# ekimb/mapquik

Hardware: AMD Instinct MI355X
Metric: Gbases/s mapped (sim CHM13v2-like HiFi, k=5 l=31 d=0.01) (higher is better)
Workload: dtype u64

## Files before the change

include/mapquik_hip_diag.h:

```cpp
#ifndef MAPQUIK_HIP_DIAG_H
#define MAPQUIK_HIP_DIAG_H

#include "mapquik_hip.h"

#ifdef __cplusplus
extern "C" {
#endif

int mq_last_map_path_counts(mq_index *idx, uint32_t *n_fast, uint32_t *n_general);

int mqdiag_last_map_spec(mq_index *idx, uint32_t *spec_id);
int mqdiag_ctx_last_map_spec(mq_ctx *ctx, uint32_t *spec_id);

int mq_last_map_order(mq_index *idx, uint32_t *n_flagged, uint32_t *n_first);

int mq_index_table_alloc_ms(mq_index *idx, float *ms);

int mq_map_launch_waves(mq_index *idx, uint32_t n_reads, uint32_t *n_waves);

int mq_map_probe_stats(mq_index *idx, const uint8_t *d_bases, const uint64_t *d_offsets, uint32_t n, uint64_t total_bases, mq_hit *d_out,
                       uint64_t *lookups, uint64_t *extra_steps);

int mq_last_read_cycles(mq_index *idx, uint32_t n, uint32_t *cycles, uint64_t *start_ticks);

int mq_probe_rate(mq_index *idx, uint32_t blocks, uint32_t per_thread, uint32_t bitmap_log2, uint32_t table_too, float *ms,
                  uint64_t *lookups, uint64_t *extra_steps);

int mq_last_stage_clocks(mq_index *idx, uint64_t *out16);

int mq_last_map_ms(mq_index *idx, float *ms);
int mq_ctx_last_map_ms(mq_ctx *ctx, float *ms);

uint64_t mqdiag_coverage_tile_bits(void);
uint64_t mqdiag_coverage_held(const mq_index *idx);
int mqdiag_coverage_ms(float *out6);

#ifdef __cplusplus
}
#endif

#endif
```

mapquik_amd/api.py:

```python
import ctypes as C
import os

import numpy as np

from . import build as _build

MQ_HIT_UNMAPPED, MQ_HIT_MAPPED, MQ_HIT_OVERFLOW = 0, 1, 2
MQ_FLAG_FOLD_CASE = 1
MQ_FLAG_FAST_KH = 2
MQ_FLAG_SEED_VARIANT_SHIFT = 8
MQ_ABI_VERSION = 4

hit_dtype = np.dtype([("status", "<u4"), ("ref_id", "<u4"), ("rc", "<u4"), ("mapq", "<u4"), ("q_start", "<u4"), ("q_end", "<u4"),
                      ("r_start", "<u4"), ("r_end", "<u4"), ("score", "<u4"), ("n_kminmers", "<u4"), ("q_start_hi", "<u4"), ("q_end_hi", "<u4")])
kminmer_dtype = np.dtype([("hash", "<u8"), ("start", "<u4"), ("end", "<u4"), ("offset", "<u4"), ("rev", "<u4")])
assert hit_dtype.itemsize == 48 and kminmer_dtype.itemsize == 24
anchor_dtype = np.dtype([("q_start", "<u4"), ("q_end", "<u4"), ("r_start", "<u4"), ("r_end", "<u4"), ("count", "<u4")])
anchor_span_dtype = np.dtype([("first", "<u4"), ("count", "<u4")])
MQ_ANCHORS_DROPPED = 0xFFFFFFFF
assert anchor_dtype.itemsize == 20 and anchor_span_dtype.itemsize == 8
chain_dtype = np.dtype([("flags", "<u4"), ("ref_id", "<u4"), ("rc", "<u4"), ("mapq", "<u4"), ("q_start", "<u4"), ("q_end", "<u4"),
                        ("r_start", "<u4"), ("r_end", "<u4"), ("score", "<u4"), ("n_runs", "<u4"), ("q_start_hi", "<u4"), ("q_end_hi", "<u4")])
chain_span_dtype = np.dtype([("first", "<u4"), ("count", "<u4")])
MQ_CHAIN_TOP = 1
# ... 104 lines not shown
    if hasattr(L, "mq_ctx_submit_fasta"):
        L.mq_host_register.argtypes = [vp, C.c_size_t]
        L.mq_host_unregister.argtypes = [vp]
        L.mq_ctx_submit_fasta.argtypes = [vp, vp, u64, u64]
        L.mq_ctx_wait_fasta.argtypes = [vp, C.POINTER(u32), C.POINTER(vp), C.POINTER(u32), C.POINTER(vp), C.POINTER(u32)]
    if hasattr(L, "mq_ctx_submit_fastx"):
        L.mq_ctx_submit_fastx.argtypes = [vp, vp, u64, u64, u32]
    if hasattr(L, "mq_ctx_wait_fasta_lines"):
        L.mq_ctx_wait_fasta_lines.argtypes = [vp, C.POINTER(u32), C.POINTER(vp), C.POINTER(vp), C.POINTER(vp), C.POINTER(vp), C.POINTER(u32)]
    if hasattr(L, "mq_index_stage_begin"):
        L.mq_index_set_table_factor.argtypes = [vp, u32]
        L.mq_index_get_params.argtypes = [vp, C.POINTER(Params)]
        L.mq_index_set_map_params.argtypes = [vp, u32, u32, u32, C.c_int]
        L.mq_index_stage_begin.argtypes = [vp, u64]
        L.mq_index_stage_piece.argtypes = [vp, u64, vp, u64, C.POINTER(u64)]
        L.mq_index_stage_done.argtypes = [vp, u64, C.c_int]
        L.mq_index_add_ref_staged.restype = C.c_int64
        L.mq_index_add_ref_staged.argtypes = [vp, u32, C.c_char_p, u64, u64, u64]
    if hasattr(L, "mq_index_add_ref_staged_lines"):
        L.mq_index_add_ref_staged_lines.restype = C.c_int64
        L.mq_index_add_ref_staged_lines.argtypes = [vp, u32, C.c_char_p, u64, u64, u64, C.POINTER(u64)]
        L.mq_index_staged_sequence.restype = C.c_int64
        L.mq_index_staged_sequence.argtypes = [vp, u64, u64, u64, vp, u64]
    L.mq_ctx_reserve.argtypes = [vp, u32, u64]
    L.mq_ctx_map_batch_device.argtypes = [vp, vp, vp, u32, u64, vp, vp]
    L.mq_ctx_last_map_ms.argtypes = [vp, C.POINTER(C.c_float)]
    L.mq_probe_rate.argtypes = [vp, u32, u32, u32, u32, C.POINTER(C.c_float), C.POINTER(u64), C.POINTER(u64)]
    L.mq_kminmers_batch.argtypes = [vp, vp, vp, u32, vp, vp, vp]
    L.mq_index_lookup.argtypes = [vp, vp, u32, vp, vp, vp]
    L.mq_format_paf.argtypes = [vp, C.c_char_p, u64, vp, C.c_char_p, C.c_size_t]
    L.mq_last_map_ms.argtypes = [vp, C.POINTER(C.c_float)]
    L.mq_last_stage_clocks.argtypes = [vp, vp]
    if hasattr(L, "mq_last_read_cycles"):
        L.mq_last_read_cycles.argtypes = [vp, u32, vp, vp]
    L.mq_map_probe_stats.argtypes = [vp, vp, vp, u32, u64, vp, C.POINTER(u64), C.POINTER(u64)]
    if hasattr(L, "mq_map_launch_waves"):
        L.mq_map_launch_waves.argtypes = [vp, u32, C.POINTER(u32)]
        L.mq_index_table_alloc_ms.argtypes = [vp, C.POINTER(C.c_float)]
    L.mq_index_save.argtypes = [vp, C.c_char_p]
    L.mq_index_clone.restype = vp
    L.mq_index_clone.argtypes = [vp, C.c_int]
    L.mq_index_load.restype = vp
    L.mq_index_load.argtypes = [C.c_char_p, C.c_int]
    L.mq_host_alloc.restype = vp
    L.mq_host_alloc.argtypes = [C.c_size_t]
    L.mq_host_free.argtypes = [vp]
    L.mq_last_map_path_counts.argtypes = [vp, C.POINTER(C.c_uint32), C.POINTER(C.c_uint32)]
    L.mq_last_map_order.argtypes = [vp, C.POINTER(C.c_uint32), C.POINTER(C.c_uint32)]
    if hasattr(L, "mq_ctx_reserve_redo"):
        L.mq_ctx_reserve_redo.argtypes = [vp, u32, u32]
        L.mq_map_reserve_redo.argtypes = [vp, u32, u32]
        L.mq_ctx_redo_counts.argtypes = [vp, C.POINTER(u32), C.POINTER(u32)]
        L.mq_map_redo_counts.argtypes = [vp, C.POINTER(u32), C.POINTER(u32)]
    pp = C.POINTER(vp)
    for kind in ("anchors", "chains"):
        if hasattr(L, "mq_ctx_reserve_" + kind):
            for scope in ("ctx", "map"):
                getattr(L, "mq_%s_reserve_%s" % (scope, kind)).argtypes = [vp, u32, u64]
                getattr(L, "mq_%s_%s" % (scope, kind)).argtypes = [vp, pp, pp, C.POINTER(u32), C.POINTER(u64), C.POINTER(u64), C.POINTER(u32)]
            getattr(L, "mq_ctx_%s_device" % kind).argtypes = [vp, pp, pp]
    if hasattr(L, "mq_format_paf_chain"):
        L.mq_format_paf_chain.argtypes = [vp, C.c_char_p, u64, vp, C.c_char_p, C.c_size_t]
    if hasattr(L, "mq_index_reopen"):
        L.mq_index_reopen.argtypes = [vp]
        L.mq_index_resize.argtypes = [vp, u64, u32]
        L.mq_index_load_sized.restype = vp
        L.mq_index_load_sized.argtypes = [C.c_char_p, C.c_int, u64, u32]
        L.mq_index_clone_sized.restype = vp
        L.mq_index_clone_sized.argtypes = [vp, C.c_int, u64, u32]
    if hasattr(L, "mq_index_merge"):
        L.mq_index_merge.argtypes = [vp, vp, u32]
        L.mq_index_merge_file.argtypes = [vp, C.c_char_p, u32]
    if hasattr(L, "mq_index_coverage"):
        L.mq_index_coverage.argtypes = [vp, C.POINTER(vp), C.POINTER(u64), C.POINTER(vp), C.POINTER(u64), C.POINTER(u64)]
        L.mq_index_coverage_release.argtypes = [vp]
        L.mqdiag_coverage_tile_bits.restype = u64
        L.mqdiag_coverage_tile_bits.argtypes = []
        L.mqdiag_coverage_held.restype = u64
        L.mqdiag_coverage_held.argtypes = [vp]
        L.mqdiag_coverage_ms.argtypes = [C.POINTER(C.c_float)]
    if hasattr(L, "mqdiag_last_map_spec"):
        L.mqdiag_last_map_spec.argtypes = [vp, C.POINTER(C.c_uint32)]
        L.mqdiag_ctx_last_map_spec.argtypes = [vp, C.POINTER(C.c_uint32)]
    if path is None:
        _lib = L
    return L


def _err(L, what):
    return MapquikError("%s: %s" % (what, (L.mq_last_error() or b"").decode(errors="replace")))


def _pooled(L, what, handle, span_dtype, item_dtype):
    sp, it = C.c_void_p(), C.c_void_p()
    n, dropped = C.c_uint32(), C.c_uint32()
    stored, needed = C.c_uint64(), C.c_uint64()
    if getattr(L, what)(handle, C.byref(sp), C.byref(it), C.byref(n), C.byref(stored), C.byref(needed), C.byref(dropped)) != 0:
        raise _err(L, what)
    spans = np.frombuffer(C.string_at(sp.value, n.value * span_dtype.itemsize), dtype=span_dtype).copy() if n.value else np.zeros(0, dtype=span_dtype)
    items = np.frombuffer(C.string_at(it.value, stored.value * item_dtype.itemsize), dtype=item_dtype).copy() if stored.value else np.zeros(0, dtype=item_dtype)
    return spans, items, dict(stored=stored.value, needed=needed.value, dropped_reads=dropped.value)


def _reserve_pooled(L, what, handle, max_reads, max_entries):
    if getattr(L, what)(handle, int(max_reads), int(max_entries)) != 0:
        raise _err(L, what)


def _pooled_device(L, what, handle):
    sp, it = C.c_void_p(), C.c_void_p()
    if getattr(L, what)(handle, C.byref(sp), C.byref(it)) != 0:
        raise _err(L, what)
    return sp.value, it.value


class PinnedBuffer:

    def __init__(self, nbytes):
        self._L = load_library()
        self._p = self._L.mq_host_alloc(nbytes)
        if not self._p:
            raise _err(self._L, "mq_host_alloc")
        self.array = np.ctypeslib.as_array((C.c_uint8 * nbytes).from_address(self._p))

    def close(self):
        if getattr(self, "_p", None):
            self.array = None
            self._L.mq_host_free(self._p)
            self._p = None

    __del__ = close


def device_count():
    return load_library().mq_device_count()


def _seq(seq):
    if isinstance(seq, (bytes, bytearray, memoryview)):
        return np.frombuffer(bytes(seq), dtype=np.uint8)
    return np.ascontiguousarray(seq, dtype=np.uint8)


def _p(a):
    return a.ctypes.data_as(C.c_void_p)


class Index:

    def __init__(self, params=None, device=0, _handle=None):
        self._L = load_library()
        self.params = params or Params()
        self._h = _handle if _handle is not None else self._L.mq_index_new(C.byref(self.params), device)
        if not self._h:
            raise _err(self._L, "mq_index_new")
        self.device = device

    def save(self, path):
        if self._L.mq_index_save(self._h, os.fsencode(path)) != 0:
            raise _err(self._L, "mq_index_save")

    @classmethod
    def load(cls, path, device=0, table_slots=0, factor=0):
        L = load_library()
        if table_slots or factor:
            h, what = L.mq_index_load_sized(os.fsencode(path), device, int(table_slots), int(factor)), "mq_index_load_sized"
# ... 183 lines not shown
        rc = self._L.mq_map_batch_device(self._h, C.c_void_p(d_bases), C.c_void_p(d_offsets), n, int(total_bases), C.c_void_p(d_out),
                                         C.c_void_p(stream))
        if rc != 0:
            raise _err(self._L, "mq_map_batch_device")

    def reserve(self, n_reads, total_bases):
        if self._L.mq_map_reserve(self._h, n_reads, int(total_bases)) != 0:
            raise _err(self._L, "mq_map_reserve")

    def reserve_redo(self, max_reads, max_read_len):
        if self._L.mq_map_reserve_redo(self._h, int(max_reads), int(max_read_len)) != 0:
            raise _err(self._L, "mq_map_reserve_redo")

    def redo_counts(self):
        a, b = C.c_uint32(), C.c_uint32()
        if self._L.mq_map_redo_counts(self._h, C.byref(a), C.byref(b)) != 0:
            raise _err(self._L, "mq_map_redo_counts")
        return a.value, b.value

    def reserve_anchors(self, max_reads, max_anchors):
        _reserve_pooled(self._L, "mq_map_reserve_anchors", self._h, max_reads, max_anchors)

    def anchors(self):
        return _pooled(self._L, "mq_map_anchors", self._h, anchor_span_dtype, anchor_dtype)

    def reserve_chains(self, max_reads, max_chains):
        _reserve_pooled(self._L, "mq_map_reserve_chains", self._h, max_reads, max_chains)

    def chains(self):
        return _pooled(self._L, "mq_map_chains", self._h, chain_span_dtype, chain_dtype)

    def format_paf_chain(self, q_id, q_len, chain):
        rec = np.zeros(1, dtype=chain_dtype)
        rec[0] = chain
        cap = 4096
        while True:
            buf = C.create_string_buffer(cap)
            w = self._L.mq_format_paf_chain(self._h, q_id.encode(), int(q_len), _p(rec), buf, cap)
            if w < 0:
                raise _err(self._L, "mq_format_paf_chain")
            if w < cap:
                return buf.value.decode()
            cap = w + 1

    def context(self):
        return Context(self)

    def last_map_ms(self):
        ms = C.c_float()
        if self._L.mq_last_map_ms(self._h, C.byref(ms)) != 0:
            raise _err(self._L, "mq_last_map_ms")
        return ms.value

    def last_stage_clocks(self):
        out = (C.c_uint64 * 16)()
        if self._L.mq_last_stage_clocks(self._h, out) != 0:
            raise _err(self._L, "mq_last_stage_clocks")
        return [int(x) for x in out]

    def probe_stats(self, d_bases, d_offsets, n, total_bases, d_out):
        a, b = C.c_uint64(), C.c_uint64()
        if self._L.mq_map_probe_stats(self._h, C.c_void_p(d_bases), C.c_void_p(d_offsets), n, int(total_bases), C.c_void_p(d_out),
                                      C.byref(a), C.byref(b)) != 0:
            raise _err(self._L, "mq_map_probe_stats")
        return a.value, b.value

    def probe_rate(self, blocks, per_thread, bitmap_log2=0, table_too=1):
        ms, a, b = C.c_float(), C.c_uint64(), C.c_uint64()
        if self._L.mq_probe_rate(self._h, blocks, per_thread, bitmap_log2, table_too, C.byref(ms), C.byref(a), C.byref(b)) != 0:
            raise _err(self._L, "mq_probe_rate")
        return ms.value, a.value, b.value

    def last_map_path_counts(self):
        a, b = C.c_uint32(), C.c_uint32()
        if self._L.mq_last_map_path_counts(self._h, C.byref(a), C.byref(b)) != 0:
            raise _err(self._L, "mq_last_map_path_counts")
        return a.value, b.value

    def last_map_spec(self):
        a = C.c_uint32()
        if self._L.mqdiag_last_map_spec(self._h, C.byref(a)) != 0:
            raise _err(self._L, "mqdiag_last_map_spec")
        return a.value

    def table_alloc_ms(self):
        ms = C.c_float()
        if self._L.mq_index_table_alloc_ms(self._h, C.byref(ms)) != 0:
            raise _err(self._L, "mq_index_table_alloc_ms")
        return ms.value

    def launch_waves(self, n_reads):
        a = C.c_uint32()
        if self._L.mq_map_launch_waves(self._h, int(n_reads), C.byref(a)) != 0:
            raise _err(self._L, "mq_map_launch_waves")
        return a.value

    def last_map_order(self):
        a, b = C.c_uint32(), C.c_uint32()
        if self._L.mq_last_map_order(self._h, C.byref(a), C.byref(b)) != 0:
            raise _err(self._L, "mq_last_map_order")
        return a.value, b.value

    def kminmers_batch(self, bases, offsets, caps=None):
        bases = _seq(bases)
        offsets = np.ascontiguousarray(offsets, dtype=np.uint64)
        n = offsets.size - 1
        if caps is None:
            caps = (offsets[1:] - offsets[:-1]).astype(np.uint64)
        koff = np.zeros(n + 1, dtype=np.uint64)
        koff[1:] = np.cumsum(np.asarray(caps, dtype=np.uint64))
        out = np.zeros(int(koff[-1]), dtype=kminmer_dtype)
        counts = np.zeros(n, dtype=np.uint32)
        if n > 0 and self._L.mq_kminmers_batch(self._h, _p(bases), _p(offsets), n, _p(koff), _p(out), _p(counts)) != 0:
            raise _err(self._L, "mq_kminmers_batch")
        res = []
        for i in range(n):
            c = int(counts[i])
            if c > int(koff[i + 1] - koff[i]):
                raise MapquikError("k-min-mer window too small for sequence %d: %d > %d" % (i, c, int(koff[i + 1] - koff[i])))
            res.append(out[int(koff[i]):int(koff[i]) + c].copy())
        return res

    def lookup(self, hashes):
        h = np.ascontiguousarray(hashes, dtype=np.uint64)
        n = h.size
        found = np.zeros(n, dtype=np.uint8)
        ent = np.zeros(n, dtype=kminmer_dtype)
        ids = np.zeros(n, dtype=np.uint32)
        if n > 0 and self._L.mq_index_lookup(self._h, _p(h), n, _p(found), _p(ent), _p(ids)) != 0:
            raise _err(self._L, "mq_index_lookup")
        return found, ent, ids

    def format_paf(self, q_id, q_len, hit):
        rec = np.zeros(1, dtype=hit_dtype)
        rec[0] = hit
        cap = 4096
        while True:
            buf = C.create_string_buffer(cap)
            w = self._L.mq_format_paf(self._h, q_id.encode(), int(q_len), _p(rec), buf, cap)
            if w < 0:
                raise _err(self._L, "mq_format_paf")
            if w < cap:
                return buf.value.decode()
            cap = w + 1

    def paf_lines(self, names, offsets, hits):
        out = []
        for i, name in enumerate(names):
            st = int(hits[i]["status"])
            if st == MQ_HIT_OVERFLOW:
                raise MapquikError("read %s: Match-run scratch overflow (raise MQ_MATCH_CAP)" % name)
            if st == MQ_HIT_MAPPED:
                out.append(self.format_paf(name, int(offsets[i + 1] - offsets[i]), hits[i]))
        return out


class Context:

    def __init__(self, index):
        self._L = index._L
        self._index = index
        self._h = self._L.mq_ctx_new(index.handle)
        if not self._h:
            raise _err(self._L, "mq_ctx_new")
        self._keep = None

# ... 40 lines not shown
            if self._L.mq_ctx_submit_fastx(self._h, _p(buf), int(begin), buf.size, 1 if fastq else 2) != 0:
                raise _err(self._L, "mq_ctx_submit_fastx")
        elif self._L.mq_ctx_submit_fasta(self._h, _p(buf), int(begin), buf.size) != 0:
            raise _err(self._L, "mq_ctx_submit_fasta")
        self._keep = (buf,)

    def wait_fasta(self):
        n, nl, fl = C.c_uint32(), C.c_uint32(), C.c_uint32()
        le, hp = C.c_void_p(), C.c_void_p()
        if self._L.mq_ctx_wait_fasta(self._h, C.byref(n), C.byref(le), C.byref(nl), C.byref(hp), C.byref(fl)) != 0:
            raise _err(self._L, "mq_ctx_wait_fasta")
        self._keep = None
        if fl.value & 1 or n.value == 0:
            return np.zeros(0, dtype=hit_dtype), np.zeros(0, dtype=np.uint32), fl.value
        hits = np.frombuffer(C.string_at(hp.value, n.value * hit_dtype.itemsize), dtype=hit_dtype).copy()
        lines = np.frombuffer(C.string_at(le.value, nl.value * 4), dtype=np.uint32).copy()
        return hits, lines, fl.value

    def wait_fasta_lines(self):
        n, fl = C.c_uint32(), C.c_uint32()
        hb, he, sl, hp = C.c_void_p(), C.c_void_p(), C.c_void_p(), C.c_void_p()
        if self._L.mq_ctx_wait_fasta_lines(self._h, C.byref(n), C.byref(hb), C.byref(he), C.byref(sl), C.byref(hp), C.byref(fl)) != 0:
            raise _err(self._L, "mq_ctx_wait_fasta_lines")
        self._keep = None
        if fl.value & 1 or n.value == 0:
            e = np.zeros(0, dtype=np.uint32)
            return np.zeros(0, dtype=hit_dtype), e, e.copy(), e.copy(), fl.value
        hits = np.frombuffer(C.string_at(hp.value, n.value * hit_dtype.itemsize), dtype=hit_dtype).copy()
        u = [np.frombuffer(C.string_at(q.value, n.value * 4), dtype=np.uint32).copy() for q in (hb, he, sl)]
        return hits, u[0], u[1], u[2], fl.value

    def wait(self):
        if self._L.mq_ctx_wait(self._h) != 0:
            raise _err(self._L, "mq_ctx_wait")
        out = self._keep[2] if self._keep else np.zeros(0, dtype=hit_dtype)
        self._keep = None
        return out

    def map_batch_device(self, d_bases, d_offsets, n, total_bases, d_out, stream=0):
        if self._L.mq_ctx_map_batch_device(self._h, C.c_void_p(d_bases), C.c_void_p(d_offsets), n, int(total_bases), C.c_void_p(d_out),
                                           C.c_void_p(stream)) != 0:
            raise _err(self._L, "mq_ctx_map_batch_device")

    def reserve_redo(self, max_reads, max_read_len):
        if self._L.mq_ctx_reserve_redo(self._h, int(max_reads), int(max_read_len)) != 0:
            raise _err(self._L, "mq_ctx_reserve_redo")

    def redo_counts(self):
        a, b = C.c_uint32(), C.c_uint32()
        if self._L.mq_ctx_redo_counts(self._h, C.byref(a), C.byref(b)) != 0:
            raise _err(self._L, "mq_ctx_redo_counts")
        return a.value, b.value

    def reserve_anchors(self, max_reads, max_anchors):
        _reserve_pooled(self._L, "mq_ctx_reserve_anchors", self._h, max_reads, max_anchors)

    def anchors(self):
        return _pooled(self._L, "mq_ctx_anchors", self._h, anchor_span_dtype, anchor_dtype)

    def reserve_chains(self, max_reads, max_chains):
        _reserve_pooled(self._L, "mq_ctx_reserve_chains", self._h, max_reads, max_chains)

    def chains(self):
        return _pooled(self._L, "mq_ctx_chains", self._h, chain_span_dtype, chain_dtype)

    def chains_device(self):
        return _pooled_device(self._L, "mq_ctx_chains_device", self._h)

    def anchors_device(self):
        return _pooled_device(self._L, "mq_ctx_anchors_device", self._h)

    def last_map_ms(self):
        ms = C.c_float()
        if self._L.mq_ctx_last_map_ms(self._h, C.byref(ms)) != 0:
            raise _err(self._L, "mq_ctx_last_map_ms")
        return ms.value

    def last_map_spec(self):
        a = C.c_uint32()
        if self._L.mqdiag_ctx_last_map_spec(self._h, C.byref(a)) != 0:
            raise _err(self._L, "mqdiag_ctx_last_map_spec")
        return a.value


def format_coverage_bed(index, refs, intervals):
    out = []
    for r in refs:
        name = index.ref_info(int(r["ref_id"]))[0].encode()
        a = int(r["first_interval"])
        for iv in intervals[a:a + int(r["n_intervals"])]:
            out.append(b"%s\t%d\t%d\n" % (name, int(iv["start"]), int(iv["end"])))
    return b"".join(out)


def format_coverage_tsv(index, refs):
    out = [b"#ref\tlen\tlive_kminmers\tcovered\tfraction\tintervals\n"]
    for r in refs:
        name = index.ref_info(int(r["ref_id"]))[0].encode()
        out.append(b"%s\t%d\t%d\t%d\t%.6f\t%d\n" % (name, int(r["len"]), int(r["live_kminmers"]), int(r["covered_bases"]),
                                                    int(r["covered_bases"]) / int(r["len"]), int(r["n_intervals"])))
    return b"".join(out)


def ref_extract(ref_idx, inp_seq_raw, params, mers_index, name=None):
    assert params is mers_index.params or bytes(params) == bytes(mers_index.params)
    return mers_index.add_ref(ref_idx, name if name is not None else str(ref_idx), inp_seq_raw)


def find_matches(q_id, q_len, q_str, ref_map, mers_index, params):
    s = _seq(q_str)
    assert q_len == s.size
    hits = mers_index.map_batch(s, np.array([0, s.size], dtype=np.uint64))
    lines = mers_index.paf_lines([q_id], [0, s.size], hits)
    return lines[0] if lines else None
```

mapquik_amd/csrc/mq_capi_diag.hpp:

```cpp
#pragma once

__global__ void probe_rate_kernel(const Bucket *__restrict__ table, uint64_t mask, uint32_t per_thread, uint64_t seed,
                                  unsigned long long *__restrict__ acc, const uint32_t *__restrict__ bitmap, uint64_t bit_mask,
                                  uint32_t table_too) {
    const uint64_t tid = (uint64_t)blockIdx.x * blockDim.x + threadIdx.x;
    const uint64_t nb = (mask + 1) >> 1;
    unsigned long long found = 0, steps = 0;
    auto mix = [](uint64_t z) {
        z += 0x9e3779b97f4a7c15ULL;
        z = (z ^ (z >> 30)) * 0xbf58476d1ce4e5b9ULL;
        z = (z ^ (z >> 27)) * 0x94d049bb133111ebULL;
        return z ^ (z >> 31);
    };
    for (uint32_t j = 0; j < per_thread; j += 4) {
        uint64_t key[4];
        uint4 kk[4];
        uint32_t bw[4];
#pragma unroll
        for (int u = 0; u < 4; ++u) {
            key[u] = mix(seed + tid * per_thread + j + u) | 1ull;
            if (bitmap) bw[u] = bitmap[(key[u] & bit_mask) >> 5];
            else kk[u] = ld_u4(&table[(key[u] & mask) >> 1].key[0]);
        }
        if (bitmap) {
// ... 6 lines not shown
        }
#pragma unroll
        for (int u = 0; u < 4; ++u) {
            const uint32_t w0 = (uint32_t)(key[u] & mask) & 1u;
            uint64_t ka = u64_of(kk[u].x, kk[u].y), kb = u64_of(kk[u].z, kk[u].w);
            uint64_t kh = w0 ? kb : ka, kp = w0 ? ka : kb;
            uint64_t b = (key[u] & mask) >> 1;
            bool hit = kh == key[u], go = !hit && kh != 0;
            if (go) {
                steps++;
                hit = kp == key[u];
                go = !hit && kp != 0;
            }
            while (go) {
                b = b + 1 == nb ? 0 : b + 1;
                const uint4 v = ld_u4(&table[b].key[0]);
                ka = u64_of(v.x, v.y);
                kb = u64_of(v.z, v.w);
                steps++;
                hit = ka == key[u];
                go = !hit && ka != 0;
                if (go) {
                    steps++;
                    hit = kb == key[u];
                    go = !hit && kb != 0;
                }
            }
            if (hit) found += table[b].pay[0].start & 1u;
        }
    }
    for (int d = 32; d >= 1; d >>= 1) {
        found += __shfl_xor(found, d, 64);
        steps += __shfl_xor(steps, d, 64);
    }
    if ((threadIdx.x & 63) == 0) {
        atomicAdd(&acc[0], found);
        atomicAdd(&acc[1], steps);
    }
}

static hipError_t counter_field(const mq_ctx *c, void *dst, size_t offset, size_t bytes) {
    return hipMemcpy(dst, reinterpret_cast<const uint8_t *>(c->d_counter.p) + offset, bytes, hipMemcpyDeviceToHost);
}

extern "C" {

int mq_last_map_path_counts(mq_index *idx, uint32_t *n_fast, uint32_t *n_general) {
    return guarded([&]() -> int {
        if (!idx || !n_fast || !n_general) return set_err(MQ_EINVAL, "bad arguments");
        std::lock_guard<std::mutex> lk(idx->mu);
        mq_ctx *c = idx->def_ctx.get();
        if (!c->ev_valid) return set_err(MQ_ESTATE, "no map launch recorded");
        int rc = use_device(idx);
        if (rc) return rc;
        HIPCHK(hipEventSynchronize(c->ev1));
        uint32_t v[2] = {0, 0};
        static_assert(offsetof(MapCounters, n_general) == offsetof(MapCounters, n_fast) + sizeof(MapCounters::n_fast), "n_fast, n_general");
        HIPCHK(counter_field(c, v, offsetof(MapCounters, n_fast), sizeof(MapCounters::n_fast) + sizeof(MapCounters::n_general)));
        *n_fast = v[0];
        *n_general = v[1];
        return MQ_OK;
    });
}

int mqdiag_last_map_spec(mq_index *idx, uint32_t *spec_id) {
    return guarded([&]() -> int {
        if (!idx || !spec_id) return set_err(MQ_EINVAL, "bad arguments");
        std::lock_guard<std::mutex> lk(idx->mu);
        mq_ctx *c = idx->def_ctx.get();
        if (!c->ev_valid) return set_err(MQ_ESTATE, "no map launch recorded");
        *spec_id = c->last_spec;
        return MQ_OK;
    });
}
int mqdiag_ctx_last_map_spec(mq_ctx *ctx, uint32_t *spec_id) {
    return guarded([&]() -> int {
        if (!ctx || !spec_id) return set_err(MQ_EINVAL, "bad arguments");
        if (!ctx->ev_valid) return set_err(MQ_ESTATE, "no map launch recorded");
        *spec_id = ctx->last_spec;
        return MQ_OK;
    });
}

int mq_last_map_order(mq_index *idx, uint32_t *n_flagged, uint32_t *n_first) {
    return guarded([&]() -> int {
        if (!idx || !n_flagged || !n_first) return set_err(MQ_EINVAL, "bad arguments");
        std::lock_guard<std::mutex> lk(idx->mu);
        mq_ctx *c = idx->def_ctx.get();
        if (!c->ev_valid) return set_err(MQ_ESTATE, "no map launch recorded");
        int rc = use_device(idx);
        if (rc) return rc;
        HIPCHK(hipEventSynchronize(c->ev1));
        uint32_t v = 0;
        HIPCHK(counter_field(c, &v, offsetof(MapCounters, n_flagged), sizeof(MapCounters::n_flagged)));
        *n_flagged = v;
        *n_first = v < WORK_FRONT_CAP ? v : WORK_FRONT_CAP;
        return MQ_OK;
    });
}

int mq_index_table_alloc_ms(mq_index *idx, float *ms) {
    return guarded([&]() -> int {
        if (!idx || !ms) return set_err(MQ_EINVAL, "bad arguments");
        std::lock_guard<std::mutex> lk(idx->mu);
        if (!idx->finalized) return set_err(MQ_ESTATE, "index not finalized");
        *ms = (float)idx->table_alloc_ms;
        return MQ_OK;
    });
}

int mq_map_launch_waves(mq_index *idx, uint32_t n_reads, uint32_t *n_waves) {
    return guarded([&]() -> int {
        if (!idx || !n_waves) return set_err(MQ_EINVAL, "bad arguments");
        int rc = use_device(idx);
        if (rc) return rc;
        if ((rc = ensure_geometry(idx))) return rc;
        *n_waves = fused_grid(idx, n_reads) * (uint32_t)MAP_WAVES;
        return MQ_OK;
    });
}

int mq_map_probe_stats(mq_index *idx, const uint8_t *d_bases, const uint64_t *d_offsets, uint32_t n, uint64_t total_bases, mq_hit *d_out,
                       uint64_t *lookups, uint64_t *extra_steps) {
    return guarded([&]() -> int {
        if (!idx || !lookups || !extra_steps) return set_err(MQ_EINVAL, "bad arguments");
        std::lock_guard<std::mutex> lk(idx->mu);
        mq_ctx *c = idx->def_ctx.get();
        int rc = ctx_map_device(c, d_bases, d_offsets, n, total_bases, d_out, nullptr, true);
        if (rc) return rc;
        HIPCHK(hipEventSynchronize(c->ev1));
        ProbeStats v;
        HIPCHK(counter_field(c, &v, offsetof(MapCounters, probe), sizeof(MapCounters::probe)));
        *extra_steps = v.steps;
        *lookups = v.lookups;
        return MQ_OK;
    });
}

int mq_last_read_cycles(mq_index *idx, uint32_t n, uint32_t *cycles, uint64_t *start_ticks) {
    return guarded([&]() -> int {
        if (!idx || !cycles || !start_ticks) return set_err(MQ_EINVAL, "bad arguments");
        std::lock_guard<std::mutex> lk(idx->mu);
        mq_ctx *c = idx->def_ctx.get();
        if (!c->ev_valid || n > c->reads_cap) return set_err(MQ_ESTATE, "no instrumented launch of that size recorded");
        int rc = use_device(idx);
        if (rc) return rc;
        HIPCHK(hipEventSynchronize(c->ev1));
        HIPCHK(hipMemcpy(cycles, ctx_read_cycles(c), (size_t)n * sizeof(uint32_t), hipMemcpyDeviceToHost));
        HIPCHK(hipMemcpy(start_ticks, ctx_read_start(c), (size_t)n * sizeof(uint64_t), hipMemcpyDeviceToHost));
        return MQ_OK;
    });
}

int mq_last_stage_clocks(mq_index *idx, uint64_t *out16) {
    return guarded([&]() -> int {
        if (!idx || !out16) return set_err(MQ_EINVAL, "bad arguments");
        std::lock_guard<std::mutex> lk(idx->mu);
        mq_ctx *c = idx->def_ctx.get();
        if (!c->ev_valid) return set_err(MQ_ESTATE, "no map launch recorded");
        int rc = use_device(idx);
        if (rc) return rc;
        HIPCHK(hipEventSynchronize(c->ev1));
        static_assert(MQ_N_CLK == 16, "mq_last_stage_clocks fills 16 words (include/mapquik_hip_diag.h)");
        HIPCHK(counter_field(c, out16, offsetof(MapCounters, clk), sizeof(MapCounters::clk)));
        return MQ_OK;
    });
// ... 71 lines not shown
```

mapquik_amd/csrc/mq_capi_index.hpp:

```cpp
#pragma once

using IndexPtr = std::unique_ptr<mq_index>;

static int check_params(const mq_params *params) {
    if (!params) return set_err(MQ_EINVAL, "params is NULL");
    if (params->l < 1 || params->l > MAX_L || params->k < 1 || params->k > MAX_K) return set_err(MQ_EINVAL, "unsupported k/l: need 1 <= l <= 64 and 1 <= k <= 32");
    if (params->flags & ~(MQ_FLAG_FOLD_CASE | MQ_FLAG_FAST_KH | MQ_FLAG_SEED_VARIANT_MASK)) return set_err(MQ_EINVAL, "undefined bits in mq_params.flags");
    const uint32_t variant = (params->flags & MQ_FLAG_SEED_VARIANT_MASK) >> MQ_FLAG_SEED_VARIANT_SHIFT;
    if ((variant & MQ_SEEDVAR_POS_RUN_END) && params->l < 2)
        return set_err(MQ_EINVAL, "seeding variant 8 (position = end of the homopolymer run) needs l >= 2: the run's end is read off the window's second base");
    return MQ_OK;
}

extern "C" {

mq_index *mq_index_new(const mq_params *params, int device) {
    return guarded([&]() -> mq_index * {
        if (check_params(params) != MQ_OK) return nullptr;
        const bool init_timing = env_set("MQ_DRIVER_TIMING");
        const auto ti0 = std::chrono::steady_clock::now();
        auto stamp = [&](const char *what) {
            if (init_timing) fprintf(stderr, "    mq_index_new: +%.3f s %s\n", std::chrono::duration<double>(std::chrono::steady_clock::now() - ti0).count(), what);
        };
        int n = mq_device_count();
        stamp("hipGetDeviceCount (runtime initialised)");
        if (n <= 0) {
            set_err(MQ_ENODEVICE, "no HIP device: the mapquik HIP path has no CPU fallback");
            return nullptr;
        }
        if (device < 0 || device >= n) {
            set_err(MQ_EINVAL, "device ordinal out of range");
            return nullptr;
        }
        IndexPtr idx(new mq_index());
        idx->params = *params;
        idx->device = device;
        if (env_int("MQ_CHAIN_CHUNK", 64) == 4) idx->chain_chunk = 4;
        idx->no_spec = env_int("MQ_NO_SPEC", 0) != 0;
        set_dev_params(idx.get(), dev_params_from(*params, (params->flags & MQ_FLAG_SEED_VARIANT_MASK) >> MQ_FLAG_SEED_VARIANT_SHIFT));
        idx->force_general = env_int("MQ_FORCE_GENERAL", 0) != 0;
        idx->heavy_first = env_int("MQ_HEAVY_FIRST", 1) != 0;
        const char *pl = getenv("MQ_PIPELINE");
        idx->split = pl && strcmp(pl, "split") == 0;
        hipDeviceProp_t prop;
        if (hipSetDevice(device) != hipSuccess || hipGetDeviceProperties(&prop, device) != hipSuccess) {
            set_err(MQ_EHIP, "hipSetDevice/hipGetDeviceProperties failed");
            return nullptr;
        }
        idx->n_cu = prop.multiProcessorCount;
        stamp("hipSetDevice + hipGetDeviceProperties");
        if (alloc_table(idx.get(), 2) != MQ_OK) return nullptr;
        stamp("first hipMalloc + hipMemset (code objects loaded)");
        idx->def_ctx.reset(ctx_create(idx.get()));
        stamp("stream created");
        if (!idx->def_ctx) return nullptr;
        return idx.release();
    });
}

void mq_index_free(mq_index *idx) { delete idx; }

}


static const char *const EXTEND_FAILED = "a finalize of this reopened index failed part way: the table is no longer exact, free the index";
static const char *const MERGE_FAILED = "a merge into this index failed part way: the table is no longer exact, free the index";
static int extend_failed_err(const mq_index *idx) { return set_err(MQ_ESTATE, idx->merge_failed ? MERGE_FAILED : EXTEND_FAILED); }

static int check_new_ref(const mq_index *idx, uint32_t ref_id, uint64_t len) {
    if (idx->finalized) return set_err(MQ_ESTATE, "index already finalized");
    if (idx->extend_failed) return extend_failed_err(idx);
    if (len >= (1ull << 32)) return set_err(MQ_EINVAL, "sequence length must be < 2^32");
    if (ref_id >= MQ_MAX_REF_ID) return set_err(MQ_EINVAL, "ref_id must be < 2^24 (reference lengths are kept in a dense device array)");
    if (idx->refs.count(ref_id)) return set_err(MQ_EINVAL, "duplicate ref_id");
    return MQ_OK;
}

static uint32_t *dense_last_of(mq_index *idx) { return (idx->dp.variant & MQ_SEEDVAR_END_COMPRESSED) ? idx->bld.dense_last.p : nullptr; }

static int plan_ref_seed(mq_index *idx, const uint8_t *d_seq, uint64_t len, RefSeedArgs *A) {
    BuildScratch &b = idx->bld;
    const bool with_last = (idx->dp.variant & MQ_SEEDVAR_END_COMPRESSED) != 0;
    const uint32_t n_seg = (uint32_t)((len + REF_SEG - 1) / REF_SEG);
    double dens = idx->params.density;
    if (!(dens > 0)) dens = 0;
    if (dens > 1) dens = 1;
    uint32_t cap = (uint32_t)std::min<double>((double)REF_SEG, 3.0 * 2.0 * dens * (double)REF_SEG + 256.0);
    if (env_set("MQ_REF_CAP")) cap = (uint32_t)std::max(1, env_int("MQ_REF_CAP", 1));
    int rc;
    if ((rc = b.counts.ensure(n_seg))) return rc;
    if ((rc = b.queue.ensure(n_seg))) return rc;
    if ((rc = b.seg_off.ensure((uint64_t)n_seg + 1))) return rc;
    if (!b.info && (rc = b.info.alloc(1))) return rc;
    if (!idx->grid_ref) {
        int occ = 0;
        HIPCHK(hipOccupancyMaxActiveBlocksPerMultiprocessor(&occ, (const void *)seed_ref_kernel, 64 * SEED_WAVES, 0));
        idx->grid_ref = std::max(1, occ) * idx->n_cu;
    }
    if ((rc = b.seg_hash.ensure((uint64_t)n_seg * cap))) return rc;
    if ((rc = b.seg_pos.ensure((uint64_t)n_seg * cap))) return rc;
    if (with_last && (rc = b.seg_last.ensure((uint64_t)n_seg * cap))) return rc;
    HIPCHK(hipMemsetAsync(b.info, 0, sizeof(RefBuildInfo), 0));
    *A = RefSeedArgs{d_seq, len, n_seg, idx->dp, b.seg_hash, b.seg_pos, with_last ? b.seg_last.p : nullptr, cap, b.counts, b.queue,
                     &b.info.p->work, idx->force_general ? 1u : 0u};
    return MQ_OK;
}

static int seed_ref_segments(mq_index *idx, const RefSeedArgs &A, uint64_t *n_mz, uint32_t *n_over) {
    BuildScratch &b = idx->bld;
    int rc;
    if ((rc = launch(seed_ref_kernel, std::min<uint32_t>((uint32_t)idx->grid_ref, (A.n_seg + SEED_WAVES - 1) / SEED_WAVES), 64 * SEED_WAVES, 0, A))) return rc;
    if ((rc = launch(seed_ref_general_kernel, std::min<uint32_t>((uint32_t)idx->n_cu * 32u, A.n_seg), 64, 0, A))) return rc;
    if ((rc = launch(scan_counts_kernel, 1, 1024, 0, b.counts, A.n_seg, A.cap, b.seg_off, &b.info.p->total, b.queue))) return rc;
    RefBuildInfo h = {};
    HIPCHK(hipMemcpy(&h, b.info, offsetof(RefBuildInfo, work), hipMemcpyDeviceToHost));
    *n_mz = h.total;
    *n_over = (uint32_t)h.overflowed;
    return MQ_OK;
}

static int compact_and_redo(mq_index *idx, const RefSeedArgs &A, uint64_t n_mz, uint32_t n_over) {
// ... 361 lines not shown
```

mapquik_amd/csrc/mq_capi_map.hpp:

```cpp
#pragma once

struct LaunchOpt {
    mq_kminmer *d_dump = nullptr;
    const uint64_t *d_dump_off = nullptr;
    uint32_t *d_dump_counts = nullptr;
    MatchRec *scratch_override = nullptr;
    uint32_t cap_override = 0;
    uint32_t grid_override = 0;
    uint32_t f16 = 0;
    const uint32_t *d_lens = nullptr;
    bool instrumented = false;
    mq_ctx *outputs_of = nullptr;
    bool redo = false;
    const uint32_t *d_ids = nullptr;
    ChainRec *chain_windows_override = nullptr;
};

static int outputs_admit(const mq_ctx *c, uint32_t n) {
    int rc = c->anchors.admit(n);
    return rc ? rc : c->chains.admit(n);
}

static int launch_map(mq_ctx *c, const uint8_t *d_bases, const uint64_t *d_offsets, uint32_t n, mq_hit *d_out, hipStream_t st,
                      const LaunchOpt &o = LaunchOpt()) {
    mq_index *idx = c->idx;
    if (n == 0) return MQ_OK;
    mq_ctx *oc = o.outputs_of ? o.outputs_of : c;
    const bool delivers = !o.instrumented && !o.d_dump && !idx->split;
    const bool anch = oc->anchors.reads != 0 && delivers, chn = oc->chains.reads != 0 && delivers;
    int rc;
    if (anch && !o.redo && ((rc = oc->anchors.admit(n)) || (rc = oc->anchors.begin_batch(n, st)))) return rc;
    if (chn) {
        if (o.scratch_override && !o.chain_windows_override) return set_err(MQ_ESTATE, "a redo launch of a chains context without chain windows");
        if (!o.redo && ((rc = oc->chains.admit(n)) || (rc = oc->chains.begin_batch(n, st)))) return rc;
    }
    const auto id_map = [&o](const Buf<uint32_t> &own) -> const uint32_t * { return !o.redo ? nullptr : o.d_ids ? o.d_ids : own.p; };
    HIPCHK(hipMemsetAsync(c->d_counter, 0, sizeof(MapCounters), st));
    HIPCHK(hipEventRecord(c->ev0, st));
    MapArgs A;
    A.bases = d_bases;
    A.offsets = d_offsets;
    A.lens = o.d_lens;
    A.n = n;
    A.P = idx->dp;
    A.mz_hash = c->mz_hash;
    A.mz_pos = c->mz_pos;
    A.mz_last = c->mz_last;
    A.mz_count = c->mz_count;
    A.mz_base = c->mz_base;
    A.pool_base = c->pool_base;
    A.pool_cap = c->pool_cap;
    A.f16 = o.f16 ? o.f16 : list_f16(idx);
    A.slack = LIST_SLACK;
    A.queue = c->queue;
    A.counters = c->d_counter;
    A.force_general = idx->force_general ? 1u : 0u;
    A.table = idx->table;
    A.mask = idx->nslots - 1;
    A.ref_lens = idx->d_ref_lens;
    A.scratch_all = o.scratch_override ? o.scratch_override : c->scratch;
    A.cap_matches = o.scratch_override ? o.cap_override : idx->cap_matches;
    A.out = d_out;
    A.dump = o.d_dump;
    A.dump_off = o.d_dump_off;
    A.dump_counts = o.d_dump_counts;
    A.stats64 = &c->d_counter.p->probe;
    A.work = c->work;
    A.heavy_first = idx->heavy_first ? 1u : 0u;
    A.anchors.pool = anch ? oc->anchors.pool.p : nullptr;
    A.anchors.cap = anch ? (uint32_t)oc->anchors.cap : 0u;
    A.anchors.counters = anch ? oc->anchors.counters.p : nullptr;
    A.anchor_spans = anch ? oc->anchors.spans.p : nullptr;
    A.anchor_ids = anch ? id_map(oc->anchors.ids) : nullptr;
    if (chn) {
        ChainLaunch cl;
        cl.pool = oc->chains.pool.p;
        cl.cap = (uint32_t)oc->chains.cap;
        cl.win_cap = chain_win_cap(A.cap_matches);
        cl.counters = oc->chains.counters.p;
        cl.windows = o.scratch_override ? o.chain_windows_override : oc->chn_windows.p;
        cl.spans = oc->chains.spans.p;
        cl.ids = id_map(oc->chains.ids);
        HIPCHK(hipMemcpyAsync(&c->d_counter.p->chains, &cl, sizeof(ChainLaunch), hipMemcpyHostToDevice, st));
    }
    if (!idx->split) {
        if (n > WORK_ID_MASK) return set_err(MQ_EINVAL, "more than 2^30 - 1 reads in one batch");
        hipLaunchKernelGGL(order_reads_kernel, dim3((n + 255u) / 256u), dim3(256), 0, st, A);
        uint32_t grid = fused_grid(idx, n);
        if (o.grid_override) grid = std::min(grid, o.grid_override);
        if (anch || chn) grid = std::min(grid, idx->grid_fused_outputs);
        const dim3 blk(64 * MAP_WAVES);
        const MapPair &kp = map_pair_of(idx, o.instrumented, &c->last_spec, anch, chn);
        hipLaunchKernelGGL(kp.map, dim3(grid), blk, 0, st, A);
        HIPCHK(hipGetLastError());
        hipLaunchKernelGGL(kp.declined, dim3(grid), blk, 0, st, A);
        HIPCHK(hipGetLastError());
    } else {
        const uint32_t gs = std::min<uint32_t>(idx->grid_seed, (n + SEED_WAVES - 1) / SEED_WAVES);
        const char *ss = getenv("MQ_SEED_STOP");
        const int stop = ss ? atoi(ss) : 0;
        if (stop == 1) hipLaunchKernelGGL(seed_reads_kernel<1>, dim3(gs), dim3(64 * SEED_WAVES), 0, st, A);
        else if (stop == 2) hipLaunchKernelGGL(seed_reads_kernel<2>, dim3(gs), dim3(64 * SEED_WAVES), 0, st, A);
        else hipLaunchKernelGGL(seed_reads_kernel<0>, dim3(gs), dim3(64 * SEED_WAVES), 0, st, A);
        HIPCHK(hipGetLastError());
        const uint32_t gg = std::min<uint32_t>((uint32_t)idx->n_cu * 8u, n);
        hipLaunchKernelGGL(seed_general_kernel, dim3(gg), dim3(64), 0, st, A);
        HIPCHK(hipGetLastError());
        uint32_t gm = std::min<uint32_t>(idx->grid_map, (n + ML_WAVES - 1) / ML_WAVES);
        if (o.grid_override) gm = std::min(gm, o.grid_override);
        const dim3 blk(64 * ML_WAVES);
        if (o.instrumented) hipLaunchKernelGGL((map_lists_kernel<64, true>), dim3(gm), blk, 0, st, A);
        else if (idx->chain_chunk == 4) hipLaunchKernelGGL((map_lists_kernel<4, false>), dim3(gm), blk, 0, st, A);
        else hipLaunchKernelGGL((map_lists_kernel<64, false>), dim3(gm), blk, 0, st, A);
        HIPCHK(hipGetLastError());
    }
    HIPCHK(hipEventRecord(c->ev1, st));
    c->ev_valid = true;
    if (anch && (rc = oc->anchors.mark_done(st))) return rc;
    return chn ? oc->chains.mark_done(st) : MQ_OK;
}

static std::vector<uint32_t> overflow_reads(const mq_hit *out, uint32_t n) {
    std::vector<uint32_t> redo;
    for (uint32_t i = 0; i < n; ++i)
        if (out[i].status == MQ_HIT_OVERFLOW) redo.push_back(i);
    return redo;
}

constexpr uint32_t REDO_WAVES = (uint32_t)std::max(MAP_WAVES, ML_WAVES);
static uint32_t redo_grid(const mq_index *idx, uint32_t cap) {
    return (uint32_t)std::max<uint64_t>(1, std::min<uint64_t>(std::min(idx->grid_fused, idx->grid_map), (1ull << 30) / ((uint64_t)cap * sizeof(MatchRec) * REDO_WAVES)));
}

static int redo_relaunch(mq_ctx *c, const std::vector<uint32_t> &redo, const std::vector<uint8_t> &sb, const std::vector<uint64_t> &so, mq_hit *out) {
    mq_index *idx = c->idx;
    uint64_t sub_max = 0;
    for (size_t j = 0; j < redo.size(); ++j) sub_max = std::max(sub_max, so[j + 1] - so[j]);
    const uint64_t sub_total = so.back();
    const uint32_t cap = (uint32_t)std::max<uint64_t>(sub_max, 1);
    const uint32_t waves = REDO_WAVES;
    const uint32_t rgrid = redo_grid(idx, cap);
    int rc = ctx_ensure(c, (uint32_t)redo.size(), sub_total, 65536u);
    if (rc) return rc;
    Buf<MatchRec> big;
    Buf<ChainRec> big_chains;
    Buf<uint8_t> d_sb;
    Buf<uint64_t> d_so;
    Buf<mq_hit> d_sh;
    hipError_t e = big.try_alloc((uint64_t)rgrid * waves * cap);
    if (e == hipSuccess && c->chains.reads) e = big_chains.try_alloc((uint64_t)rgrid * waves * chain_win_cap(cap));
    if (e == hipSuccess) e = d_sb.try_alloc(sub_total + 1);
    if (e == hipSuccess) e = d_so.try_alloc(so.size());
    if (e == hipSuccess) e = d_sh.try_alloc(redo.size());
    if (e == hipSuccess && sub_total) e = hipMemcpyAsync(d_sb, sb.data(), sub_total, hipMemcpyHostToDevice, c->stream);
    if (e == hipSuccess) e = hipMemcpyAsync(d_so, so.data(), so.size() * 8, hipMemcpyHostToDevice, c->stream);
    int rrc = MQ_OK;
    std::vector<mq_hit> sh(redo.size());
    if (e == hipSuccess) {
        LaunchOpt o;
        o.scratch_override = big;
        o.cap_override = cap;
        o.grid_override = rgrid;
        o.f16 = 65536u;
        o.redo = true;
        if (c->anchors.reads) e = hipMemcpyAsync(c->anchors.ids, redo.data(), redo.size() * sizeof(uint32_t), hipMemcpyHostToDevice, c->stream);
        if (c->chains.reads && e == hipSuccess) {
            e = hipMemcpyAsync(c->chains.ids, redo.data(), redo.size() * sizeof(uint32_t), hipMemcpyHostToDevice, c->stream);
            o.chain_windows_override = big_chains;
        }
        if (e == hipSuccess) rrc = launch_map(c, d_sb, d_so, (uint32_t)redo.size(), d_sh, c->stream, o);
    }
    if (e == hipSuccess && rrc == MQ_OK) e = hipMemcpyAsync(sh.data(), d_sh, redo.size() * sizeof(mq_hit), hipMemcpyDeviceToHost, c->stream);
    if (e == hipSuccess) e = hipStreamSynchronize(c->stream);
    else hipStreamSynchronize(c->stream);
    if (e != hipSuccess) return set_err(e == hipErrorOutOfMemory ? MQ_ENOMEM : MQ_EHIP, std::string("overflow retry: ") + hipGetErrorString(e));
// ... 873 lines not shown
```

mapquik_amd/csrc/mq_host_state.hpp:

```cpp
#pragma once


constexpr uint32_t MQ_MAX_REF_ID = 1u << 24;
struct mq_index;
using RefMap = std::map<uint32_t, std::pair<std::string, uint64_t>>;

static bool env_set(const char *name) { return getenv(name) != nullptr; }
static int env_int(const char *name, int fallback) {
    const char *e = getenv(name);
    return e ? atoi(e) : fallback;
}

template <class... KA>
static int launch(void (*kernel)(KA...), uint32_t grid, uint32_t block, hipStream_t stream, std::common_type_t<KA>... args) {
    hipLaunchKernelGGL(kernel, dim3(grid), dim3(block), 0, stream, args...);
    HIPCHK(hipGetLastError());
    return MQ_OK;
}

enum class FxKind { None, Fasta, Fastq, FastaLines };

struct RedoArena;
struct mq_ctx;

template <class Item, class Span>
struct PooledOutput {
    const char *const noun, *const adjective;
    uint32_t reads = 0;
    uint64_t cap = 0;
    Buf<Item> pool;
    Buf<Span> spans;
    Buf<PoolCounters> counters;
    Buf<uint32_t> ids;
    PinnedBuf<Item> h_pool;
    PinnedBuf<Span> h_spans;
    PinnedBuf<PoolCounters> h_counters;
    ScopedEvent done;
    bool ran = false;
    uint32_t n = 0;

    PooledOutput(const char *noun_, const char *adjective_) : noun(noun_), adjective(adjective_) {}
    int admit(uint32_t batch) const {
        if (reads && batch > reads)
            return set_err(MQ_EINVAL, std::string("more reads in the batch than the context's ") + adjective + " reservation holds (mq_ctx_reserve_" + noun + ": max_reads)");
        return MQ_OK;
    }
    int begin_batch(uint32_t batch, hipStream_t st) {
        HIPCHK(hipMemsetAsync(counters, 0, sizeof(PoolCounters), st));
        n = batch;
        return MQ_OK;
    }
    int mark_done(hipStream_t st) {
        HIPCHK(hipEventRecord(done, st));
        ran = true;
        return MQ_OK;
    }
    int require_reserved() const {
        return reads ? MQ_OK : set_err(MQ_ESTATE, std::string("no ") + noun + " reserved on this context: call mq_ctx_reserve_" + noun + " first");
    }
    int device_pointers(const Span **d_spans, const Item **d_pool) const {
        if (!reads) return require_reserved();
        *d_spans = spans;
        *d_pool = pool;
        return MQ_OK;
    }
    template <class Alloc, class Commit>
    int reserve(mq_ctx *c, uint32_t max_reads, uint64_t max_entries, Alloc alloc_extra, Commit commit_extra);
    int read_back(mq_ctx *c, const Span **out_spans, const Item **out_pool, uint32_t *n_reads, uint64_t *stored, uint64_t *needed, uint32_t *dropped_reads);
};

struct mq_ctx {
    mq_index *idx = nullptr;
    ScopedStream stream;
    ScopedEvent ev0, ev1;
    bool ev_valid = false;
    uint32_t last_spec = 0;
    Buf<MapCounters> d_counter;
    Buf<MatchRec> scratch;
    size_t scratch_waves = 0;
    Buf<unsigned long long> mz_hash;
    Buf<uint32_t> mz_pos;
    Buf<uint32_t> mz_last;
    uint64_t mz_cap = 0;
    Buf<uint32_t> mz_count;
    Buf<uint64_t> mz_base;
    Buf<uint32_t> queue;
    Buf<uint4> work;
    uint64_t reads_cap = 0;
    uint64_t pool_base = 0, pool_cap = 0;
    Buf<uint8_t> st_bases;
    Buf<uint64_t> st_off;
    Buf<mq_hit> st_out;
    Buf<uint32_t> st_lens;
    PinnedBuf<uint64_t> h_off;
    PinnedBuf<mq_hit> h_out;
    Buf<uint32_t> fx_tile_counts, fx_tile_off;
    Buf<uint32_t> fx_nl;
    PinnedBuf<uint32_t> h_fx_nl;
    Buf<FxResult> fx_info;
    PinnedBuf<FxResult> h_fx_info;
    PinnedBuf<uint8_t> h_fx_tail;
    Buf<uint8_t> fl_joined;
    Buf<uint32_t> fl_hb, fl_he;
    PinnedBuf<uint32_t> h_fl_hb, h_fl_he, h_fl_lens;
    bool fl_used = false;
    FxKind fx_kind = FxKind::None;
    uint32_t fx_bytes = 0;
    bool pending = false;
    const uint8_t *p_bases = nullptr;
    const uint64_t *p_offsets = nullptr;
    const uint32_t *p_lens = nullptr;
    uint32_t p_n = 0;
    mq_hit *p_out = nullptr;
    PooledOutput<mq_anchor, mq_anchor_span> anchors{"anchors", "anchor"};
    PooledOutput<mq_chain, mq_chain_span> chains{"chains", "chains"};
    Buf<ChainRec> chn_windows;
    std::unique_ptr<RedoArena> redo;
};

struct RedoArena {
    uint32_t max_reads = 0, max_read_len = 0;
    uint64_t stride = 0;
    uint32_t cap = 0, grid = 0;
    mq_ctx sub;
    Buf<uint8_t> bases;
    Buf<uint64_t> offsets;
    Buf<uint32_t> lens, ids;
    Buf<uint64_t> src;
    Buf<mq_hit> hits;
    Buf<MatchRec> windows;
    Buf<ChainRec> chain_windows;
    Buf<RedoCounters> counters;
    ScopedEvent done;
    bool ran = false;
    uint32_t last_n = 0;
    ~RedoArena() {
        if (ran) (void)hipEventSynchronize(done);
    }
};

static const uint32_t *ctx_read_cycles(const mq_ctx *c) { return c->mz_count; }
static const uint64_t *ctx_read_start(const mq_ctx *c) { return c->mz_base; }

static void ctx_release(mq_ctx *c) {
    if (!c) return;
    if (c->stream) hipStreamSynchronize(c->stream);
    delete c;
}
struct CtxRelease {
    void operator()(mq_ctx *c) const { ctx_release(c); }
};
using CtxPtr = std::unique_ptr<mq_ctx, CtxRelease>;

struct KmmChunk {
    Buf<RefKmm> d;
    uint64_t n = 0;
};

struct BuildScratch {
    Buf<uint8_t> seq;
    Buf<unsigned long long> seg_hash;
// ... 91 lines not shown
    int err = 0;
    double ms = 0;
    bool made() const { return thread.joinable() || table; }
    void start(int device, uint64_t n) {
        nslots = n;
        thread = std::thread([this, device]() {
            hipError_t e = hipSetDevice(device);
            Buf<Bucket> t;
            const auto t0 = std::chrono::steady_clock::now();
            if (e == hipSuccess) e = t.try_alloc(table_bytes_of(nslots) / sizeof(Bucket));
            ScopedStream st;
            if (e == hipSuccess) e = hipStreamCreateWithFlags(&st.h, hipStreamNonBlocking);
            if (e == hipSuccess) e = hipMemsetAsync(t, 0, table_bytes_of(nslots), st);
            if (e == hipSuccess) e = hipStreamSynchronize(st);
            ms = std::chrono::duration<double, std::milli>(std::chrono::steady_clock::now() - t0).count();
            if (e == hipSuccess) table = std::move(t);
            err = (int)e;
        });
    }
    void join() {
        if (thread.joinable()) thread.join();
    }
    Buf<Bucket> take(uint64_t want) {
        join();
        Buf<Bucket> t = std::move(table);
        if (nslots != want || err != 0) t.reset();
        return t;
    }
    ~TableReservation() { join(); }
};

struct CoverState {
    Buf<unsigned long long> bitmap;
    Buf<uint64_t> base, lens_c;
    Buf<unsigned long long> live;
    Buf<CovTile> tiles;
    Buf<uint32_t> tile_runs;
    Buf<unsigned long long> tile_off, ref_sums, first_interval, acc;
    Buf<mq_cov_interval> intervals;
    std::vector<mq_ref_coverage> h_refs;
    std::vector<mq_cov_interval> h_intervals;
    uint64_t out_of_range = 0;
    void free_device() { reset_all(bitmap, base, lens_c, live, tiles, tile_runs, tile_off, ref_sums, first_interval, acc, intervals); }
    void drop() {
        free_device();
        std::vector<mq_ref_coverage>().swap(h_refs);
        std::vector<mq_cov_interval>().swap(h_intervals);
        out_of_range = 0;
    }
    uint64_t held() const { return h_refs.capacity() * sizeof(mq_ref_coverage) + h_intervals.capacity() * sizeof(mq_cov_interval); }
};

struct mq_index {
    mq_params params;
    DevParams dp;
    int device = 0;
    int n_cu = 0;
    std::once_flag geometry_once;
    int geometry_rc = MQ_OK;
    std::mutex mu;
    RefMap refs;
    uint64_t n_kmm_total = 0;
    bool finalized = false;
    bool extending = false;
    bool extend_failed = false;
    bool merge_failed = false;
    std::mutex ctx_mu;
    std::vector<mq_ctx *> ctxs;
    uint32_t table_factor = 0;
    uint64_t nslots = 0;
    uint64_t n_unique = 0, n_keys = 0;
    int grid_ref = 0;
    uint32_t grid_fused = 0, grid_seed = 0, grid_map = 0;
    std::once_flag outputs_geometry_once;
    int outputs_geometry_rc = MQ_OK;
    uint32_t grid_fused_outputs = 0;
    uint32_t cap_matches = 0;
    bool split = false;
    bool force_general = false;
    bool heavy_first = true;
    int chain_chunk = 64;
    bool no_spec = false;
    uint32_t map_spec = 0;
    double t_add_ms = 0;
    double table_alloc_ms = 0;
    CtxPtr def_ctx;
    CoverState cov;
    Buf<uint64_t> d_ref_lens;
    Buf<Bucket> table;
    BuildScratch bld;
    StageState stage;
    std::vector<KmmChunk> chunks;
    TableReservation rsv;

    ~mq_index() {
        rsv.join();
        hipSetDevice(device);
    }
};

constexpr uint64_t MQ_MAX_TABLE_SLOTS = 1ull << 40;
static uint64_t table_slots_at(uint64_t factor, uint64_t n_kmm) {
    const uint64_t want = n_kmm > MQ_MAX_TABLE_SLOTS ? 2 * MQ_MAX_TABLE_SLOTS : factor * n_kmm;
    uint64_t nslots = 1024;
    while (nslots < want && nslots <= MQ_MAX_TABLE_SLOTS) nslots <<= 1;
    return nslots;
}
static uint64_t table_slots_for(const mq_index *idx, uint64_t n_kmm) {
    const int lf = env_int("MQ_TABLE_FACTOR", 0);
    const uint64_t factor = lf >= 2 ? (uint64_t)lf : idx->table_factor ? (uint64_t)idx->table_factor : 8ull;
    return table_slots_at(factor, n_kmm);
}

static int sized_table_slots(uint64_t table_slots, uint32_t slots_per_kminmer, uint64_t n_kmm, uint64_t n_keys, uint64_t *out) {
    *out = 0;
    if (table_slots && slots_per_kminmer) return set_err(MQ_EINVAL, "table size: table_slots or slots_per_kminmer, not both");
    if (table_slots) {
        if (table_slots < 2 || (table_slots & (table_slots - 1)) != 0 || table_slots > MQ_MAX_TABLE_SLOTS)
            return set_err(MQ_EINVAL, "table_slots: a power of two in [2, 2^40]");
        if (table_slots <= n_keys) return set_err(MQ_EINVAL, "table_slots: more slots than the index has keys (a table needs an empty slot)");
        *out = table_slots;
    } else if (slots_per_kminmer) {
        if (slots_per_kminmer < 2 || slots_per_kminmer > 64) return set_err(MQ_EINVAL, "slots per k-min-mer: 2..64");
        uint64_t s = table_slots_at(slots_per_kminmer, n_kmm);
        while (s <= n_keys && s <= MQ_MAX_TABLE_SLOTS) s <<= 1;
        if (s > MQ_MAX_TABLE_SLOTS) return set_err(MQ_EINVAL, "slots per k-min-mer: the table would pass 2^40 slots");
        *out = s;
    }
    return MQ_OK;
}

extern "C" {

const char *mq_last_error(void) { return g_err.c_str(); }
int mq_abi_version(void) { return MQ_ABI_VERSION; }

int mq_device_count(void) {
    int n = 0;
    hipError_t e = hipGetDeviceCount(&n);
    if (e != hipSuccess) {
        set_err(MQ_ENODEVICE, std::string("hipGetDeviceCount: ") + hipGetErrorString(e));
        return 0;
    }
    return n;
}

void mq_params_default(mq_params *p) {
    p->k = 5;
    p->l = 31;
    p->density = 0.01;
    p->use_hpc = 1;
    p->c = 4;
    p->s = 11;
    p->g = 2000;
    p->flags = 0;
}

}

static uint64_t density_bound(double density, uint32_t variant) {
    if (variant & MQ_SEEDVAR_HASH32) {
        if (variant & MQ_SEEDVAR_F32_BOUND) {
            const float f = (float)density * 4294967295.0f;
            if (!(f > 0.0f)) return 0;
            if (f >= 4294967296.0f) return 0xFFFFFFFFull;
            return (uint64_t)(uint32_t)f;
// ... 6 lines not shown
    if (variant & MQ_SEEDVAR_F32_BOUND) {
        const float f = (float)density * 18446744073709551615.0f;
        if (!(f > 0.0f)) return 0;
        if (f >= 18446744073709551616.0f) return UINT64_MAX;
        return (uint64_t)f;
    }
    const double d = density * 18446744073709551615.0;
    if (!(d > 0.0)) return 0;
    if (d >= 18446744073709551616.0) return UINT64_MAX;
    return (uint64_t)d;
}
static void set_dev_bound(DevParams &dp, double density, uint32_t variant) {
    uint64_t b = density_bound(density, variant);
    dp.keep_none = 0;
    if (variant & MQ_SEEDVAR_STRICT_BOUND) {
        if (b == 0) dp.keep_none = 1;
        else b -= 1;
    }
    if (variant & MQ_SEEDVAR_HASH32) b = (b & 0xFFFFFFFFull) | (b << 32);
    dp.bound = b;
    dp.variant = variant;
}

static DevParams dev_params_from(const mq_params &p, uint32_t variant) {
    DevParams dp{};
    set_dev_bound(dp, p.density, variant);
    dp.k = p.k;
    dp.l = p.l;
    dp.use_hpc = p.use_hpc ? 1 : 0;
    dp.c = p.c;
    dp.s = p.s;
    dp.g = p.g;
    dp.fold = (p.flags & MQ_FLAG_FOLD_CASE) ? 1u : 0u;
    dp.fast_kh = (p.flags & MQ_FLAG_FAST_KH) ? 1u : 0u;
    return dp;
}

static int use_device(const mq_index *idx) {
    HIPCHK(hipSetDevice(idx->device));
    return MQ_OK;
}

static uint32_t bucket_walk_grid(uint64_t nb1) { return (uint32_t)std::min<uint64_t>((2 * nb1 + 255) / 256, 1u << 16); }
static uint32_t slot_array_grid(uint64_t n) { return (uint32_t)std::min<uint64_t>((n + 255) / 256, 1u << 16); }
static uint32_t ahead_grid(uint64_t n) { return (uint32_t)std::max<uint64_t>(1, std::min<uint64_t>((n + 256 * RETABLE_AHEAD - 1) / (256 * RETABLE_AHEAD), 1u << 16)); }

static int new_table(Buf<Bucket> &table, uint64_t nslots) {
    int rc = table.alloc(table_bytes_of(nslots) / sizeof(Bucket));
    if (rc) return rc;
    HIPCHK(hipMemsetAsync(table, 0, table_bytes_of(nslots), 0));
    return MQ_OK;
}
static int alloc_table(mq_index *idx, uint64_t nslots) {
    if (nslots < 2) nslots = 2;
    const auto t0 = std::chrono::steady_clock::now();
    int rc = new_table(idx->table, nslots);
    if (rc) return rc;
    HIPCHK(hipDeviceSynchronize());
    idx->table_alloc_ms = std::chrono::duration<double, std::milli>(std::chrono::steady_clock::now() - t0).count();
    idx->nslots = nslots;
    return MQ_OK;
}

using MapFn = void (*)(MapArgs);
struct MapPair {
    MapFn map, declined;
};
template <int CH, bool TIMING, bool VAR, class Spec = SpecNone, bool ANCH = false, bool CHN = false>
constexpr MapPair map_pair() {
    return {map_kernel<CH, TIMING, VAR, Spec, ANCH, CHN>, map_declined_kernel<CH, TIMING, VAR, Spec, ANCH, CHN>};
}
static const MapPair MAP_KERNELS[2][2][2] = {{{map_pair<64, false, false>(), map_pair<4, false, false>()}, {map_pair<64, true, false>(), map_pair<64, true, false>()}},
                                             {{map_pair<64, false, true>(), map_pair<4, false, true>()}, {map_pair<64, true, true>(), map_pair<64, true, true>()}}};
template <bool ANCH, bool CHN>
constexpr MapPair out_pair(bool var, bool ch4) {
    return var ? (ch4 ? map_pair<4, false, true, SpecNone, ANCH, CHN>() : map_pair<64, false, true, SpecNone, ANCH, CHN>())
               : (ch4 ? map_pair<4, false, false, SpecNone, ANCH, CHN>() : map_pair<64, false, false, SpecNone, ANCH, CHN>());
}
#define MQ_OUT_PAIRS(A, C) {{out_pair<A, C>(false, false), out_pair<A, C>(false, true)}, {out_pair<A, C>(true, false), out_pair<A, C>(true, true)}}
static const MapPair MAP_KERNELS_OUTPUTS[2][2][2][2] = {{{{{nullptr, nullptr}, {nullptr, nullptr}}, {{nullptr, nullptr}, {nullptr, nullptr}}}, MQ_OUT_PAIRS(false, true)},
                                                        {MQ_OUT_PAIRS(true, false), MQ_OUT_PAIRS(true, true)}};
#undef MQ_OUT_PAIRS

struct MapSpec {
    uint32_t k, l, use_hpc, fold, fast_kh;
    MapPair pair;
};
template <class S>
constexpr MapSpec map_spec() {
    return {S::K, S::L, S::HPC ? 1u : 0u, S::FOLD ? 1u : 0u, S::FAST_KH ? 1u : 0u, map_pair<64, false, false, S>()};
}
static const MapSpec MAP_SPECS[] = {map_spec<SpecFixed<5, 31, true, false>>(), map_spec<SpecFixed<7, 31, true, false>>(),
                                    map_spec<SpecFixed<5, 31, true, true>>()};
constexpr uint32_t N_MAP_SPECS = sizeof(MAP_SPECS) / sizeof(MAP_SPECS[0]);

static bool spec_matches(const MapSpec &s, const DevParams &dp, bool any_fold) {
    return s.k == dp.k && s.l == dp.l && s.use_hpc == dp.use_hpc && s.fast_kh == dp.fast_kh && (any_fold || s.fold == dp.fold);
}
static bool specs_allowed(const mq_index *idx) { return !idx->no_spec && idx->dp.variant == 0 && idx->chain_chunk != 4; }
static uint32_t map_spec_of(const mq_index *idx) {
    if (!specs_allowed(idx)) return 0;
    for (uint32_t i = 0; i < N_MAP_SPECS; ++i)
        if (spec_matches(MAP_SPECS[i], idx->dp, false)) return i + 1;
    return 0;
}
static const MapPair &map_pair_of(const mq_index *idx, bool instrumented, uint32_t *spec_id = nullptr, bool anchors = false, bool chains = false) {
    if ((anchors || chains) && !instrumented) {
        if (spec_id) *spec_id = 0;
        return MAP_KERNELS_OUTPUTS[anchors][chains][idx->dp.variant != 0][idx->chain_chunk == 4];
    }
    const uint32_t sid = instrumented ? 0u : idx->map_spec;
    if (spec_id) *spec_id = sid;
    return sid ? MAP_SPECS[sid - 1].pair : MAP_KERNELS[idx->dp.variant != 0][instrumented][idx->chain_chunk == 4];
}
static void set_dev_params(mq_index *idx, const DevParams &dp) {
    idx->dp = dp;
    idx->map_spec = map_spec_of(idx);
}

static int occ_of(const void *fn, int threads, int &occ) {
    HIPCHK(hipOccupancyMaxActiveBlocksPerMultiprocessor(&occ, fn, threads, 0));
    if (occ < 1) occ = 1;
    if (occ > 8) occ = 8;
    const int oe = env_int("MQ_OCC", 0);
    if (oe >= 1 && oe < occ) occ = oe;
    return MQ_OK;
}
static int ensure_geometry_once(mq_index *idx) {
    int occ = 0, occ_min = INT_MAX, rc;
    std::vector<MapPair> pairs = {map_pair_of(idx, true), MAP_KERNELS[idx->dp.variant != 0][0][idx->chain_chunk == 4]};
    if (specs_allowed(idx))
        for (const MapSpec &s : MAP_SPECS)
            if (spec_matches(s, idx->dp, true)) pairs.push_back(s.pair);
    for (const MapPair &kp : pairs)
        for (const MapFn fn : {kp.map, kp.declined}) {
            if ((rc = occ_of((const void *)fn, 64 * MAP_WAVES, occ))) return rc;
            occ_min = std::min(occ_min, occ);
        }
    idx->grid_fused = (uint32_t)(occ_min * idx->n_cu);
    if ((rc = occ_of((const void *)seed_reads_kernel<0>, 64 * SEED_WAVES, occ))) return rc;
    idx->grid_seed = (uint32_t)(occ * idx->n_cu);
    if ((rc = occ_of((const void *)map_lists_kernel<64, false>, 64 * ML_WAVES, occ))) return rc;
    idx->grid_map = (uint32_t)(occ * idx->n_cu);
    idx->cap_matches = (uint32_t)env_int("MQ_MATCH_CAP", 2048);
    if (idx->cap_matches < 1) idx->cap_matches = 1;
    return MQ_OK;
}

static uint32_t fused_grid(const mq_index *idx, uint32_t n) { return std::min<uint32_t>(idx->grid_fused, (n + MAP_WAVES - 1) / MAP_WAVES); }

static uint32_t fx_grid(const mq_index *idx, uint32_t n_tiles) { return std::max<uint32_t>(1, std::min<uint32_t>((n_tiles + 3) / 4, (uint32_t)idx->n_cu * 8u)); }

static int ensure_geometry(mq_index *idx) {
    std::call_once(idx->geometry_once, [idx] { idx->geometry_rc = ensure_geometry_once(idx); });
    return idx->geometry_rc;
}

static int ensure_outputs_geometry(mq_index *idx) {
    int rc = ensure_geometry(idx);
    if (rc) return rc;
    std::call_once(idx->outputs_geometry_once, [idx] {
        int occ = 0, occ_min = INT_MAX;
        for (const MapPair *kp : {&map_pair_of(idx, false, nullptr, true, false), &map_pair_of(idx, false, nullptr, false, true), &map_pair_of(idx, false, nullptr, true, true)})
            for (const MapFn fn : {kp->map, kp->declined}) {
                if ((idx->outputs_geometry_rc = occ_of((const void *)fn, 64 * MAP_WAVES, occ))) return;
                occ_min = std::min(occ_min, occ);
            }
        idx->grid_fused_outputs = std::min(idx->grid_fused, (uint32_t)(occ_min * idx->n_cu));
    });
    return idx->outputs_geometry_rc;
}

static uint32_t chain_win_cap(uint32_t cap) { return std::max(cap, MAP_LDS_RECS); }
static size_t map_waves_for(const mq_index *idx, uint32_t n) {
    const size_t max_waves = std::max((size_t)idx->grid_fused * MAP_WAVES, (size_t)idx->grid_map * ML_WAVES);
    const size_t wpw = (size_t)std::max(MAP_WAVES, ML_WAVES);
    return std::min(max_waves, ((size_t)n + wpw - 1) / wpw * wpw + wpw);
}

static uint32_t list_f16(const mq_index *idx) {
    double d = idx->params.density;
    if (!(d > 0)) d = 0;
    double f = 4.0 * d + 1.0 / 512.0;
    if (f > 1.0) f = 1.0;
    const int e = env_int("MQ_LIST_F16", -1);
    if (e >= 0) return (uint32_t)std::min(65536, e);
    return (uint32_t)std::ceil(f * 65536.0);
}
constexpr uint32_t LIST_SLACK = 64;

static int ctx_ensure(mq_ctx *c, uint32_t n, uint64_t total_bases, uint32_t f16) {
    mq_index *idx = c->idx;
    int rc = ensure_geometry(idx);
    if (rc) return rc;
    if (!c->d_counter && (rc = c->d_counter.alloc(1))) return rc;
    if (!c->ev0) {
        HIPCHK(hipEventCreate(&c->ev0.h));
        HIPCHK(hipEventCreate(&c->ev1.h));
    }
    {
        const size_t max_waves = std::max((size_t)idx->grid_fused * MAP_WAVES, (size_t)idx->grid_map * ML_WAVES);
        const size_t want = map_waves_for(idx, n);
        if (want > c->scratch_waves) {
            c->scratch_waves = 0;
            const size_t nw = std::min(max_waves, want + want / 4);
            if ((rc = c->scratch.alloc(nw * idx->cap_matches))) return rc;
            c->scratch_waves = nw;
        }
    }
    if (n > c->reads_cap) {
        c->reads_cap = 0;
        reset_all(c->mz_count, c->mz_base, c->queue, c->work);
        const uint64_t nc = (uint64_t)n + n / 4 + 64;
        if ((rc = c->mz_count.alloc(nc)) || (rc = c->mz_base.alloc(nc)) || (rc = c->queue.alloc(nc)) || (rc = c->work.alloc(nc + WORK_FRONT_CAP))) {
            reset_all(c->mz_count, c->mz_base, c->queue, c->work);
            return rc;
        }
        c->reads_cap = nc;
    }
    const uint64_t regular = ((total_bases * f16) >> 16) + (uint64_t)LIST_SLACK * n + 64;
    const uint64_t pool = f16 >= 65536u ? 0 : std::max<uint64_t>(regular / 8, 1ull << 20);
    const uint64_t need = regular + pool;
    c->pool_base = regular;
    c->pool_cap = pool;
    if (need > c->mz_cap) {
        c->mz_cap = 0;
        reset_all(c->mz_hash, c->mz_pos, c->mz_last);
        const uint64_t nc = need + need / 8;
        if ((rc = c->mz_hash.alloc(nc)) || (rc = c->mz_pos.alloc(nc)) || ((idx->dp.variant & MQ_SEEDVAR_END_COMPRESSED) && (rc = c->mz_last.alloc(nc)))) {
            reset_all(c->mz_hash, c->mz_pos, c->mz_last);
            return rc;
        }
        c->mz_cap = nc;
    }
    return MQ_OK;
}

static mq_ctx *ctx_create(mq_index *idx) {
    mq_ctx *c = new (std::nothrow) mq_ctx();
    if (!c) {
        set_err(MQ_ENOMEM, "out of host memory");
        return nullptr;
    }
    c->idx = idx;
    if (hipSetDevice(idx->device) != hipSuccess || hipStreamCreateWithFlags(&c->stream.h, hipStreamNonBlocking) != hipSuccess) {
        set_err(MQ_EHIP, "hipStreamCreate failed");
        c->stream.h = nullptr;
        ctx_release(c);
        return nullptr;
    }
    return c;
}

static uint32_t max_ref_id(const RefMap &refs) { return refs.empty() ? 0 : refs.rbegin()->first; }
static std::vector<uint64_t> dense_ref_lens(const RefMap &refs) {
    std::vector<uint64_t> lens((size_t)max_ref_id(refs) + 1, 0);
    for (auto &kv : refs) lens[kv.first] = kv.second.second;
    return lens;
}
static int upload_ref_lens(const RefMap &refs, Buf<uint64_t> &d_lens) {
    const std::vector<uint64_t> lens = dense_ref_lens(refs);
    int rc = d_lens.alloc(lens.size());
    if (rc) return rc;
    HIPCHK(hipMemcpy(d_lens, lens.data(), lens.size() * sizeof(uint64_t), hipMemcpyHostToDevice));
    return MQ_OK;
}
static int upload_ref_lens(mq_index *idx) { return upload_ref_lens(idx->refs, idx->d_ref_lens); }

static void free_build_scratch(mq_index *idx) {
    idx->stage.reset();
    idx->bld = BuildScratch();
}
```

mapquik_amd/csrc/mq_map_kernels.hpp:

```cpp
#pragma once


struct MapArgs {
    const uint8_t *bases;
    const uint64_t *offsets;
    const uint32_t *lens;
    uint32_t n;
    DevParams P;
    unsigned long long *mz_hash;
    uint32_t *mz_pos;
    uint32_t *mz_last;
    uint32_t *mz_count;
    uint64_t *mz_base;
    uint64_t pool_base, pool_cap;
    uint32_t f16, slack;
    uint32_t *queue;
    MapCounters *counters;
    uint32_t force_general;
    const Bucket *table;
    uint64_t mask;
    const uint64_t *ref_lens;
    MatchRec *scratch_all;
    uint32_t cap_matches;
    mq_hit *out;
    mq_kminmer *dump;
    const uint64_t *dump_off;
    uint32_t *dump_counts;
    ProbeStats *stats64;
    uint4 *work;
    uint32_t heavy_first;
    AnchorOut anchors;
    mq_anchor_span *anchor_spans;
    const uint32_t *anchor_ids;
};

__device__ __forceinline__ uint32_t *read_cycles(const MapArgs &A) { return A.mz_count; }
__device__ __forceinline__ uint64_t *read_start(const MapArgs &A) { return A.mz_base; }

constexpr uint32_t WORK_FRONT_CAP = 32768;
constexpr uint32_t WORK_SKIP = 0x80000000u, WORK_TOO_LONG = 0x40000000u, WORK_ID_MASK = 0x3FFFFFFFu;

__device__ __forceinline__ bool window_periodic(const uint8_t *p) {
    uint32_t by[12];
#pragma unroll
    for (int j = 0; j < 3; ++j) {
        const uint4 v = *reinterpret_cast<const uint4_unaligned *>(p + 16 * j);
        const uint32_t w[4] = {v.x, v.y, v.z, v.w};
#pragma unroll
        for (int i = 0; i < 4; ++i) by[4 * j + i] = ((((w[i] >> 1) & 0x03030303u) * 0x01041040u) >> 24);
    }
    const uint64_t s0 = (uint64_t)(by[0] | (by[1] << 8) | (by[2] << 16) | (by[3] << 24)) | ((uint64_t)(by[4] | (by[5] << 8) | (by[6] << 16) | (by[7] << 24)) << 32);
    const uint64_t s1 = (uint64_t)(by[8] | (by[9] << 8) | (by[10] << 16) | (by[11] << 24));
    bool hit = false;
#pragma unroll
    for (uint32_t lag = 1; lag <= 16; ++lag) {
        const uint64_t sh = (s0 >> (2u * lag)) | (s1 << (64u - 2u * lag));
        const uint64_t d = s0 ^ sh;
        hit |= __popcll((d | (d >> 1)) & 0x5555555555555555ull) <= 5;
    }
    return hit;
}

__global__ __launch_bounds__(256) void order_reads_kernel(const MapArgs A) {
    const uint32_t r = blockIdx.x * 256u + threadIdx.x;
    if (r >= A.n) return;
    const uint64_t o0 = A.offsets[r];
    const uint64_t len = A.lens ? (uint64_t)A.lens[r] : A.offsets[r + 1] - o0;
    uint32_t w = r;
    if (len >> 32) w |= WORK_TOO_LONG;
    else if (A.heavy_first && len >= 512u) {
        const uint32_t ln = (uint32_t)len;
        auto win = [&](uint32_t at) { return A.bases + ((o0 + at) & ~(uint64_t)63); };
        const bool p1 = window_periodic(win(ln / 6u)), p2 = window_periodic(win(ln / 2u)), p3 = window_periodic(win((ln / 6u) * 5u));
        if (p1 | p2 | p3) {
            const uint32_t k = atomicAdd(&A.counters->n_flagged, 1u);
            if (k < WORK_FRONT_CAP) {
                A.work[WORK_FRONT_CAP - 1u - k] = make_uint4((uint32_t)o0, (uint32_t)(o0 >> 32), ln, w);
                w |= WORK_SKIP;
            }
        }
    }
    A.work[WORK_FRONT_CAP + r] = make_uint4((uint32_t)o0, (uint32_t)(o0 >> 32), (uint32_t)len, w);
}

__device__ __forceinline__ void list_region(const MapArgs &A, uint64_t o0_rel, uint64_t len, uint32_t r, uint64_t &base, uint32_t &cap) {
    base = ((o0_rel * A.f16) >> 16) + (uint64_t)A.slack * r;
    const uint64_t c = ((len * A.f16) >> 16) + A.slack;
    cap = c > 0xFFFFFFF0ull ? 0xFFFFFFF0u : (uint32_t)c;
}
constexpr uint32_t LIST_OVERFLOW = 0xFFFFFFFEu;
__device__ __forceinline__ bool pool_take(const MapArgs &A, uint32_t cnt, uint64_t &base) {
    unsigned long long at = 0;
    if (lane_id() == 0) at = atomicAdd(&A.counters->pool_cursor, (unsigned long long)cnt);
    at = rdlane64(at, 0);
    base = A.pool_base + at;
    return at + cnt <= A.pool_cap;
}

template <int STOP = 0, bool VAR = true, class Spec = SpecNone>
__device__ __forceinline__ uint32_t seed_read_fast(const MapArgs &A, const SeedTables &T, SeedLds &S, const uint8_t *seq,
                                                   uint32_t len, uint64_t &base, uint32_t cap, uint32_t &n_moved, APre &pre, bool pre_valid) {
    uint32_t cnt = seed_sequence_fast<STOP, false, VAR, Spec>(seq, len, A.P, T, S, A.mz_hash + base, A.mz_pos + base, cap, pre, pre_valid, SeedView(),
                                                        A.mz_last ? A.mz_last + base : nullptr);
    if (cnt != SD_NOT_FAST && cnt > cap) {
        if (pool_take(A, cnt, base)) {
            seed_sequence_fast<0, false, VAR, Spec>(seq, len, A.P, T, S, A.mz_hash + base, A.mz_pos + base, cnt, pre, false, SeedView(), A.mz_last ? A.mz_last + base : nullptr);
            n_moved++;
        } else {
            cnt = LIST_OVERFLOW;
        }
    }
    return cnt;
}

template <bool VAR = true>
__device__ __forceinline__ uint32_t seed_read_general(const MapArgs &A, WaveLds &S, const uint8_t *seq, uint64_t len, uint64_t &base,
                                                      uint32_t cap, uint32_t &n_moved) {
    uint32_t cnt;
    {
        SoaListSink sink(A.mz_hash + base, A.mz_pos + base, (VAR && A.mz_last) ? A.mz_last + base : nullptr, cap);
        uint32_t mz_count = 0;
        seed_segment<VAR>(seq, len, 0, len, A.P, S, sink, mz_count);
        cnt = sink.written;
    }
    if (cnt > cap) {
        if (pool_take(A, cnt, base)) {
            SoaListSink sink(A.mz_hash + base, A.mz_pos + base, (VAR && A.mz_last) ? A.mz_last + base : nullptr, cnt);
            uint32_t mz_count = 0;
            seed_segment<VAR>(seq, len, 0, len, A.P, S, sink, mz_count);
            n_moved++;
        } else {
            cnt = LIST_OVERFLOW;
        }
    }
    return cnt;
}

constexpr uint32_t HYB_MIN_CLEAN = 2048;
struct CleanPiece {
    uint4 v[4];
};
__device__ __forceinline__ void clean_request(const uint8_t *__restrict__ seq, uint64_t len, uint64_t p, CleanPiece &c) {
    const uint64_t at = p + 64u * lane_id();
#pragma unroll
    for (int j = 0; j < 4; ++j) c.v[j] = make_uint4(0u, 0u, 0u, 0u);
    if (at + 64u <= len) {
#pragma unroll
        for (int j = 0; j < 4; ++j) c.v[j] = *reinterpret_cast<const uint4_unaligned *>(seq + at + 16 * j);
    }
}
__device__ __forceinline__ uint64_t clean_blocks(const CleanPiece &c, uint64_t len, uint64_t p, bool fold) {
    const uint64_t at = p + 64u * lane_id();
    bool ok = false;
    if (at + 64u <= len) {
        const uint32_t fm = fold ? 0xDFDFDFDFu : 0xFFFFFFFFu;
        uint32_t all = 0x80808080u;
#pragma unroll
        for (int j = 0; j < 4; ++j) {
            const uint32_t w[4] = {c.v[j].x, c.v[j].y, c.v[j].z, c.v[j].w};
#pragma unroll
            for (int i = 0; i < 4; ++i) {
                const uint32_t x = w[i] & fm;
                uint32_t is = 0;
#pragma unroll
                for (int t = 0; t < 4; ++t) {
                    const uint32_t y = x ^ (t == 0 ? 0x41414141u : t == 1 ? 0x43434343u : t == 2 ? 0x47474747u : 0x54545454u);
                    is |= ~(((y & 0x7F7F7F7Fu) + 0x7F7F7F7Fu) | y | 0x7F7F7F7Fu);
                }
                all &= is;
            }
        }
        ok = all == 0x80808080u;
    }
    return __ballot(ok);
}
__device__ __forceinline__ bool next_clean_stretch(const uint8_t *__restrict__ seq, uint64_t len, uint64_t from, bool fold, uint64_t &s, uint64_t &d) {
    constexpr uint64_t NONE = ~(uint64_t)0;
    uint64_t run_s = NONE;
    CleanPiece cur, nxt;
    if (from < len) clean_request(seq, len, from, cur);
    for (uint64_t p = from; p < len; p += 4096u) {
        if (p + 4096u < len) clean_request(seq, len, p + 4096u, nxt);
        const uint64_t m = clean_blocks(cur, len, p, fold);
        cur = nxt;
        uint32_t bit = 0;
        while (bit < 64u) {
            if (run_s == NONE) {
                const uint64_t rest = m >> bit;
                if (!rest) break;
// ... 83 lines not shown
            V.first_prev = 4u;
            if (s > 0) {
                uint32_t b = seq[s - 1];
                if (spec_fold<Spec>(P) && b - 'a' < 26u) b -= 32u;
                V.first_prev = b == 'A' ? 0u : b == 'C' ? 1u : b == 'T' ? 2u : b == 'G' ? 3u : 4u;
            }
            V.elig_end = (uint32_t)(((d - s) + 127u) & ~(uint64_t)63);
            V.pos_add = (uint32_t)s;
            V.more_after = 0u;
            const uint32_t left = cap_ > n_out ? cap_ - n_out : 0u;
            charge(0);
            const uint32_t c = seed_sequence_fast<0, true, VAR, Spec>(seq + s, (uint32_t)(d - s), P, T, SF, A.mz_hash + base_ + n_out, A.mz_pos + base_ + n_out, left, pre, false, V,
                                                                A.mz_last ? A.mz_last + base_ + n_out : nullptr);
            asm volatile("s_waitcnt vmcnt(0)" ::: "memory");
            wave_sync();
            charge(1);
            if (c == SD_NOT_FAST) {
                seg_a = s;
                seg_min_last = 0;
            } else {
                n_out += c;
                seg_a = heads_back<Spec>(seq, s, d, spec_l<Spec>(P) - 1u, P);
                seg_min_last = d;
            }
        }
        if (seg_a < len && seg_min_last < len) general(seg_a, len, seg_min_last);
        charge(0);
        return n_out;
    };
    uint32_t cnt = 0, cap_now = cap;
    for (int attempt = 0;; ++attempt) {
        cnt = pass(base, cap_now);
        if (cnt <= cap_now || attempt == 1) break;
        if (!pool_take(A, cnt, base)) {
            cnt = LIST_OVERFLOW;
            break;
        }
        cap_now = cnt;
        n_moved++;
    }
    return cnt;
}

#ifndef MQ_ML_NB
#define MQ_ML_NB 6
#endif
constexpr int ML_NB = MQ_ML_NB;
constexpr uint32_t ML_LIST_CAP = 64 * ML_NB + MAX_L;
static_assert(MAX_L >= 32, "k - 1 <= 31 entries of overlap between chunks");
struct MapListLds {
    unsigned long long h[ML_LIST_CAP];
    uint32_t p[ML_LIST_CAP];
    MatchRec rec[MAP_LDS_RECS];
};

__device__ __forceinline__ void store_hit(const MapArgs &A, uint32_t r, const mq_hit &h) {
    if (lane_id() == 0) {
        A.out[r] = h;
        if (A.dump_counts) A.dump_counts[r] = h.n_kminmers;
    }
}

typedef uint2 __attribute__((aligned(8))) span_word;
static_assert(sizeof(mq_anchor_span) == 8 && sizeof(mq_anchor) == 20, "anchor records");
__device__ __forceinline__ void store_span(const MapArgs &A, uint32_t r, const mq_anchor_span &sp) {
    if (lane_id() == 0) {
        const uint32_t id = A.anchor_ids ? A.anchor_ids[r] : r;
        if (id != 0xFFFFFFFFu) *reinterpret_cast<span_word *>(A.anchor_spans + id) = make_uint2(sp.first, sp.count);
    }
}

static_assert(sizeof(mq_chain_span) == 8, "chain span");
__device__ __forceinline__ void store_chain_span(const MapArgs &A, uint32_t r, const mq_chain_span &sp) {
    if (lane_id() == 0) {
        const ChainLaunch &C = A.counters->chains;
        const uint32_t id = C.ids ? C.ids[r] : r;
        if (id != 0xFFFFFFFFu) *reinterpret_cast<span_word *>(C.spans + id) = make_uint2(sp.first, sp.count);
    }
}
__device__ __forceinline__ ChainRec *chain_window(const MapArgs &A, uint32_t wave_gid) {
    return A.counters->chains.windows + (size_t)wave_gid * A.counters->chains.win_cap;
}

template <int CH, bool TIMING, bool VAR = true, class Spec = SpecNone, bool ANCH = false, bool CHN = false>
__device__ __forceinline__ void map_read(const MapArgs &A, MapListLds &S, MatchRec *scratch, uint32_t r, uint64_t len, uint32_t cnt,
                                         uint64_t base, unsigned long long &t_steps, unsigned long long &t_lookups, mq_hit &h,
                                         mq_anchor_span *sp = nullptr, ChainRec *cwin = nullptr, mq_chain_span *csp = nullptr) {
    const uint32_t lane = lane_id();
    const DevParams &P = A.P;
    const uint32_t k = spec_k<Spec>(P);
    h.status = MQ_HIT_UNMAPPED;
    h.ref_id = h.rc = h.mapq = h.q_start = h.q_end = h.r_start = h.r_end = h.score = h.n_kminmers = h.q_start_hi = h.q_end_hi = 0;
    if constexpr (ANCH) sp->first = sp->count = 0;
    if constexpr (CHN) csp->first = csp->count = 0;
    uint32_t n_kmm = 0;
    if (cnt == LIST_OVERFLOW) {
        h.status = MQ_HIT_OVERFLOW;
    } else if (cnt >= k) {
        mq_kminmer *d = nullptr;
        uint32_t dcap = 0;
        if (A.dump) {
            d = A.dump + A.dump_off[r];
            dcap = (uint32_t)(A.dump_off[r + 1] - A.dump_off[r]);
        }
        MapSink sink(A.table, A.mask, P, scratch, A.cap_matches, S.rec, d, dcap, var_rev_eq<VAR>(P));
        const unsigned long long *lh = A.mz_hash + base;
        const uint32_t *lp = A.mz_pos + base;
        const uint32_t chunk = 64u * (uint32_t)ML_NB + k - 1u;
        for (uint32_t g = 0; g + k <= cnt;) {
            const uint32_t have = cnt - g < chunk ? cnt - g : chunk;
            {
                unsigned long long hv[ML_NB + 1];
                uint32_t pv[ML_NB + 1];
#pragma unroll
                for (int j = 0; j <= ML_NB; ++j) {
                    const uint32_t i = lane + 64u * (uint32_t)j;
                    hv[j] = 0;
                    pv[j] = 0;
                    if (i < have) {
                        hv[j] = ld_sc1_u64(lh + g + i);
                        pv[j] = ld_sc1_u32(lp + g + i);
                    }
                }
#pragma unroll
                for (int j = 0; j <= ML_NB; ++j) {
                    const uint32_t i = lane + 64u * (uint32_t)j;
                    if (i < have) {
                        S.h[i] = hv[j];
                        S.p[i] = pv[j];
                    }
                }
            }
            wave_sync();
            mq_clk(5);
            uint32_t *mzq = (VAR && A.mz_last) ? reinterpret_cast<uint32_t *>(S.h) : nullptr;
            sink.template consume_list<ML_NB, Spec>(S.h, S.p, have, [&]() {
                if (mzq) {
                    const uint32_t *lq = A.mz_last + base + g;
                    wave_sync();
                    for (uint32_t i = lane; i < have; i += 64u) mzq[i] = ld_sc1_u32(lq + i);
                    wave_sync();
                }
            }, mzq);
            wave_sync();
            g += have - (k - 1u);
        }
        sink.finish_runs();
        n_kmm = sink.kmm_count;
        if (sink.n_matches > 0 && sink.n_matches <= MAP_LDS_RECS && sink.n_matches <= (uint32_t)CH) {
            wave_sync();
            MatchRec m0 = {};
            if (lane_id() < sink.n_matches) m0 = S.rec[lane_id()];
            mq_clk(8);
            if constexpr (CHN) chain_stage<CH, ANCH, true>(S.rec, sink.n_matches, P, len, A.ref_lens, h, &m0, &A.anchors, sp, &A.counters->chains, cwin, csp);
            else if constexpr (ANCH) chain_stage<CH, true>(S.rec, sink.n_matches, P, len, A.ref_lens, h, &m0, &A.anchors, sp);
            else chain_stage<CH>(S.rec, sink.n_matches, P, len, A.ref_lens, h, &m0);
        } else {
            if (sink.n_matches > 0 && sink.n_matches <= A.cap_matches) {
                wave_sync();
                sink.records_to_scratch();
            }
            if (sink.n_matches > A.cap_matches) {
                h.status = MQ_HIT_OVERFLOW;
            } else if (sink.n_matches > 0) {
                asm volatile("s_waitcnt vmcnt(0)" ::: "memory");
                wave_sync();
                mq_clk(8);
                if constexpr (CHN) chain_stage<CH, ANCH, true>(scratch, sink.n_matches, P, len, A.ref_lens, h, nullptr, &A.anchors, sp, &A.counters->chains, cwin, csp);
                else if constexpr (ANCH) chain_stage<CH, true>(scratch, sink.n_matches, P, len, A.ref_lens, h, nullptr, &A.anchors, sp);
                else chain_stage<CH>(scratch, sink.n_matches, P, len, A.ref_lens, h);
            }
        }
        if (TIMING) {
            t_steps += wave_sum_u32(sink.probe_steps);
            t_lookups += n_kmm;
        }
    }
    h.n_kminmers = n_kmm;
    mq_clk(9);
}

#ifndef MQ_MAP_WAVES
#define MQ_MAP_WAVES 8
#endif
#ifndef MQ_MAP_MIN_WAVES
#define MQ_MAP_MIN_WAVES 4
#endif
constexpr int MAP_WAVES = MQ_MAP_WAVES;

union MapWaveLds {
    SeedLds seed;
    WaveLds general;
    MapListLds map;
};

template <int CH, bool TIMING = false, bool VAR = false, class Spec = SpecNone, bool ANCH = false, bool CHN = false>
__global__ __launch_bounds__(64 * MAP_WAVES, MQ_MAP_MIN_WAVES) void map_kernel(const MapArgs A) {
    __shared__ struct {
        SeedTables T;
        MapWaveLds SS[MAP_WAVES];
    } W;
    SeedTables &T = W.T;
    MapWaveLds(&SS)[MAP_WAVES] = W.SS;
    build_seed_tables(T, spec_l<Spec>(A.P), var_h32<VAR>(A.P));
    __syncthreads();
    const uint32_t lane = lane_id();
    const uint32_t wv = rdfirst(threadIdx.x >> 6);
    MapWaveLds &S = SS[wv];
    const size_t wave_gid = (size_t)blockIdx.x * MAP_WAVES + wv;
    MatchRec *scratch = A.scratch_all + wave_gid * A.cap_matches;
    const DevParams &P = A.P;
    const uint64_t o_base = A.offsets[0];
    uint32_t n_fast = 0, n_general = 0, n_moved = 0;
    unsigned long long t_steps = 0, t_lookups = 0;
#ifdef MQ_STAGE_CLOCKS
    if (lane == 0)
        for (int i = 0; i < MQ_N_CLK; ++i) mq_clk_lds().acc[wv][i] = 0;
    mq_clk(-1);
#endif
    const uint32_t nf = A.counters->n_flagged < WORK_FRONT_CAP ? A.counters->n_flagged : WORK_FRONT_CAP;
    const uint4 *work = A.work + (WORK_FRONT_CAP - nf);
    const uint32_t n_items = A.n + nf;
    uint32_t r = 0xFFFFFFFFu;
    uint64_t o0 = 0, len = 0;
    const uint32_t n_waves = gridDim.x * (uint32_t)MAP_WAVES;
    uint32_t own1 = (uint32_t)wave_gid, own2 = n_waves + (uint32_t)wave_gid;
    auto take_now = [&]() {
        for (;;) {
            uint32_t i;
            if (own1 != 0xFFFFFFFFu) {
                i = own1;
                own1 = 0xFFFFFFFFu;
            } else if (own2 != 0xFFFFFFFFu) {
                i = own2;
                own2 = 0xFFFFFFFFu;
            } else {
                i = 0;
                if (lane == 0) i = atomicAdd(&A.counters->seed_work, 1u);
                i = rdfirst(i) + 2u * n_waves;
            }
            r = 0xFFFFFFFFu;
            if (i >= n_items) return;
            const uint4 d = work[i];
            if (d.w & WORK_SKIP) continue;
            r = d.w & WORK_ID_MASK;
            o0 = ((uint64_t)d.y << 32) | d.x;
            len = (uint64_t)d.z | ((uint64_t)((d.w >> 30) & 1u) << 32);
            return;
        }
    };
    take_now();
    APre pre;
    while (r < A.n) {
        const unsigned long long t_read0 = TIMING ? __builtin_amdgcn_s_memtime() : 0ull;
        const unsigned long long t_real0 = TIMING ? __builtin_amdgcn_s_memrealtime() : 0ull;
        uint32_t rn_v = own2;
        if (own2 == 0xFFFFFFFFu) {
            if (lane == 0) rn_v = atomicAdd(&A.counters->seed_work, 1u);
            rn_v += 2u * n_waves;
        }
        own2 = 0xFFFFFFFFu;
        uint32_t cnt = 0;
        uint64_t base = 0;
        mq_clk(11);
        if (len >> 32) {
            cnt = LIST_OVERFLOW;
        } else if (len >= (uint64_t)spec_l<Spec>(P) + spec_k<Spec>(P) - 1u && !var_keep_none<VAR>(P)) {
            uint32_t cap;
            list_region(A, o0 - o_base, len, r, base, cap);
            cnt = A.force_general ? SD_NOT_FAST : seed_read_fast<0, VAR, Spec>(A, T, S.seed, A.bases + o0, (uint32_t)len, base, cap, n_moved, pre, false);
            if (cnt == SD_NOT_FAST) {
                n_general++;
                if (lane == 0) A.queue[atomicAdd(&A.counters->queue_len, 1u)] = r;
                cnt = 0;
                mq_clk(10);
            } else {
                n_fast++;
            }
            asm volatile("s_waitcnt vmcnt(0)" ::: "memory");
            wave_sync();
            mq_clk(4);
        }
        const uint32_t rn = rdfirst(rn_v);
        uint4 nd = make_uint4(0u, 0u, 0u, 0u);
        if (lane == 0 && rn < n_items) nd = work[rn];
        mq_hit h;
        mq_anchor_span sp;
        mq_chain_span csp;
        if constexpr (CHN) map_read<CH, TIMING, VAR, Spec, ANCH, true>(A, S.map, scratch, r, len, cnt, base, t_steps, t_lookups, h, &sp, chain_window(A, wave_gid), &csp);
        else if constexpr (ANCH) map_read<CH, TIMING, VAR, Spec, true>(A, S.map, scratch, r, len, cnt, base, t_steps, t_lookups, h, &sp);
        else map_read<CH, TIMING, VAR, Spec>(A, S.map, scratch, r, len, cnt, base, t_steps, t_lookups, h);
        wave_sync();
        const uint32_t r_done = r;
        const uint32_t nw = rdfirst(nd.w);
        o0 = ((uint64_t)rdfirst(nd.y) << 32) | rdfirst(nd.x);
        len = (uint64_t)rdfirst(nd.z) | ((uint64_t)((nw >> 30) & 1u) << 32);
        r = rn < n_items ? (nw & WORK_ID_MASK) : 0xFFFFFFFFu;
        asm volatile("" ::: "memory");
        store_hit(A, r_done, h);
        if constexpr (ANCH) store_span(A, r_done, sp);
        if constexpr (CHN) store_chain_span(A, r_done, csp);
        if (rn < n_items && (nw & WORK_SKIP)) take_now();
        if (TIMING && lane == 0) {
            const unsigned long long dt = __builtin_amdgcn_s_memtime() - t_read0;
            read_cycles(A)[r_done] = dt > 0xFFFFFFFFull ? 0xFFFFFFFFu : (uint32_t)dt;
            read_start(A)[r_done] = t_real0;
        }
    }
    if (lane == 0) {
        if (n_fast) atomicAdd(&A.counters->n_fast, n_fast);
        if (n_general) atomicAdd(&A.counters->n_general, n_general);
        if (n_moved) atomicAdd(&A.counters->n_moved, n_moved);
        if (TIMING) {
            atomicAdd(&A.stats64->steps, t_steps);
            atomicAdd(&A.stats64->lookups, t_lookups);
        }
#ifdef MQ_STAGE_CLOCKS
        for (int i = 0; i < MQ_N_CLK; ++i) atomicAdd(&A.counters->clk[i], mq_clk_lds().acc[wv][i]);
#endif
    }
}

template <int CH, bool TIMING = false, bool VAR = false, class Spec = SpecNone, bool ANCH = false, bool CHN = false>
__global__ __launch_bounds__(64 * MAP_WAVES, MQ_MAP_MIN_WAVES) void map_declined_kernel(const MapArgs A) {
    const uint32_t nq = A.counters->queue_len;
    if (nq == 0) return;
    __shared__ struct {
        SeedTables T;
        MapWaveLds SS[MAP_WAVES];
    } W;
    build_seed_tables(W.T, spec_l<Spec>(A.P), var_h32<VAR>(A.P));
    __syncthreads();
    const uint32_t lane = lane_id();
    const uint32_t wv = rdfirst(threadIdx.x >> 6);
    MapWaveLds &S = W.SS[wv];
    const size_t wave_gid = (size_t)blockIdx.x * MAP_WAVES + wv;
    MatchRec *scratch = A.scratch_all + wave_gid * A.cap_matches;
    const uint64_t o_base = A.offsets[0];
    uint32_t n_moved = 0;
    unsigned long long t_steps = 0, t_lookups = 0;
    for (;;) {
        uint32_t i = 0;
        if (lane == 0) i = atomicAdd(&A.counters->declined_work, 1u);
        i = rdfirst(i);
        if (i >= nq) break;
        const uint32_t r = A.queue[i];
        const unsigned long long t_read0 = TIMING ? __builtin_amdgcn_s_memtime() : 0ull;
        const unsigned long long t_real0 = TIMING ? __builtin_amdgcn_s_memrealtime() : 0ull;
        const uint64_t o0 = A.offsets[r];
        const uint64_t len = A.lens ? (uint64_t)A.lens[r] : A.offsets[r + 1] - o0;
        uint64_t base;
        uint32_t cap;
        list_region(A, o0 - o_base, len, r, base, cap);
        unsigned long long tacc[3] = {0ull, 0ull, 0ull};
        const uint32_t cnt = seed_read_hybrid<VAR, Spec>(A, W.T, S.seed, S.general, A.bases + o0, len, base, cap, n_moved, TIMING ? tacc : nullptr);
        asm volatile("s_waitcnt vmcnt(0)" ::: "memory");
        wave_sync();
        mq_hit h;
        mq_anchor_span sp;
        mq_chain_span csp;
        if constexpr (CHN) map_read<CH, TIMING, VAR, Spec, ANCH, true>(A, S.map, scratch, r, len, cnt, base, t_steps, t_lookups, h, &sp, chain_window(A, wave_gid), &csp);
        else if constexpr (ANCH) map_read<CH, TIMING, VAR, Spec, true>(A, S.map, scratch, r, len, cnt, base, t_steps, t_lookups, h, &sp);
        else map_read<CH, TIMING, VAR, Spec>(A, S.map, scratch, r, len, cnt, base, t_steps, t_lookups, h);
        wave_sync();
        store_hit(A, r, h);
        if constexpr (ANCH) store_span(A, r, sp);
        if constexpr (CHN) store_chain_span(A, r, csp);
        if (TIMING && lane == 0) {
            const unsigned long long dt = __builtin_amdgcn_s_memtime() - t_read0;
            read_cycles(A)[r] = dt > 0xFFFFFFFFull ? 0xFFFFFFFFu : (uint32_t)dt;
            auto u21 = [](unsigned long long c) { return (c >> 8) > 0x1FFFFFull ? 0x1FFFFFull : (c >> 8); };
            read_start(A)[r] = (1ull << 63) | u21(tacc[0]) | (u21(tacc[1]) << 21) | (u21(tacc[2]) << 42);
            (void)t_real0;
// ... 126 lines not shown
```

mapquik_amd/csrc/mq_probe.hpp:

```cpp
#pragma once
#include <hip/hip_runtime.h>
#include <stdint.h>

#include "../../include/mapquik_hip.h"
#include "mq_device.hpp"
#include "mq_hash.hpp"
#include "mq_wave.hpp"

namespace mq {

__device__ __forceinline__ uint4 ld_u4(const void *p) { return *reinterpret_cast<const uint4 *>(p); }
__device__ __forceinline__ uint64_t u64_of(uint32_t lo, uint32_t hi) { return ((uint64_t)hi << 32) | lo; }
__device__ __forceinline__ bool probe_table(const Bucket *__restrict__ table, uint64_t mask, uint64_t key, Entry &out) {
    const uint64_t nb = (mask + 1) >> 1;
    if (key == 0) {
        out = table[nb].pay[0];
        return entry_live(out);
    }
    const uint64_t s0 = key & mask;
    uint64_t b = s0 >> 1;
    uint32_t w = (uint32_t)s0 & 1u;
    for (uint32_t step = 0;; ++step) {
        const unsigned long long k = table[b].key[w];
        if (k == key) {
// ... 158 lines not shown
        const uint32_t id_p = (uint32_t)__builtin_amdgcn_update_dpp((int)c_id, (int)r_id, 0x138, 0xf, 0xf, false);
        const uint32_t off_p = (uint32_t)__builtin_amdgcn_update_dpp((int)c_off, (int)e.offset, 0x138, 0xf, 0xf, false);
        const bool both = hit && hit_p;
        const bool cf = both && ((int32_t)(e.offset - off_p) == 1);
        const bool cr = both && r_id == id_p && srel == 1u && ((int32_t)(off_p - e.offset) == 1);
        const uint32_t sv = srel ? 2u : 1u;
        const bool nonconst = cf && srel == 1u;
        uint32_t sigma = hit ? sv : 0u;
        if (__ballot(nonconst)) {
            const uint64_t constmask = __ballot(!nonconst);
            const uint64_t constF = __ballot(!nonconst && hit && sv == 1u);
            const uint64_t lt_mask = lane ? (~0ull >> (64u - lane)) : 0ull;
            const uint64_t below = constmask & lt_mask;
            const bool baseF = below ? ((constF >> (63 - __clzll((long long)below))) & 1ull) != 0 : (c_sigma == 1u);
            if (nonconst) sigma = baseF ? 1u : 2u;
        }
        const uint32_t sigma_p = (uint32_t)__builtin_amdgcn_update_dpp((int)c_sigma, (int)sigma, 0x138, 0xf, 0xf, false);
        const bool prevF = sigma_p == 1u, prevR = sigma_p == 2u;
        const bool isnew = hit && !((prevF && cf) || (prevR && cr));
        const uint64_t hitmask = __ballot(hit);
        const uint64_t newmask = __ballot(isnew);
        const bool cont0 = (hitmask & 1ull) && !(newmask & 1ull);
        if (c_open && n > 0 && !cont0) {
            if (lane == 0) put_rec(n_matches, M);
            n_matches++;
            c_open = false;
        }
        if (n > 0) {
            const uint64_t next_breaks = ((~hitmask | newmask) >> 1);
            const bool is_end = hit && lane + 1u < n && ((next_breaks >> lane) & 1ull);
            const uint64_t endmask = __ballot(is_end);
            const uint64_t below = newmask & ((lane >= 63u) ? ~0ull : ((2ull << lane) - 1ull));
            const int fl = below ? 63 - __clzll((long long)below) : -1;
            const int src = fl < 0 ? 0 : fl;
            const uint32_t f_qs = (uint32_t)__shfl((int)q_start, src, 64);
            const uint32_t f_rs = (uint32_t)__shfl((int)e.start, src, 64);
            const uint32_t f_re = (uint32_t)__shfl((int)e.end, src, 64);
            const uint32_t f_id = (uint32_t)__shfl((int)r_id, src, 64);
            const uint32_t f_rc = (uint32_t)__shfl((int)srel, src, 64);
            MatchRec m;
            if (fl >= 0) {
                m.q_start = f_qs;
                m.rc = f_rc;
                m.ref = f_id;
                m.count = lane - (uint32_t)fl + 1u;
                m.r_start = f_rc ? e.start : f_rs;
                m.r_end = f_rc ? f_re : e.end;
            } else {
                m.q_start = M.q_start;
                m.rc = M.rc;
                m.ref = M.ref;
                m.count = M.count + lane + 1u;
                m.r_start = M.rc ? e.start : M.r_start;
                m.r_end = M.rc ? M.r_end : e.end;
            }
            m.q_end = q_end;
            m.done = 0;
            if (is_end) {
                const uint32_t mi = n_matches + mbcnt64(endmask);
                put_rec(mi, m);
            }
            n_matches += (uint32_t)__popcll(endmask);
            const int last = (int)n - 1;
            c_hit = (uint32_t)((hitmask >> last) & 1ull);
            c_id = rdlane(r_id, last);
            c_off = rdlane(e.offset, last);
            c_sigma = rdlane(sigma, last);
            if (c_hit) {
                M.q_start = rdlane(m.q_start, last);
                M.q_end = rdlane(m.q_end, last);
                M.r_start = rdlane(m.r_start, last);
                M.r_end = rdlane(m.r_end, last);
                M.count = rdlane(m.count, last);
                M.ref = rdlane(m.ref, last);
                M.rc = rdlane(m.rc, last);
                M.done = 0;
                c_open = true;
            } else {
                c_open = false;
            }
        }
    }

    template <int NB, class Spec = SpecNone, class F>
    __device__ __forceinline__ void consume_list(const unsigned long long *mzh, const uint32_t *mzp, uint32_t have, const F &hashes_done,
                                                 const uint32_t *mzq = nullptr) {
        const uint32_t k = spec_k<Spec>(P), l = spec_l<Spec>(P);
        if (have < k) return;
        const uint32_t lane = lane_id();
        const uint32_t K = have - k + 1u;
        uint64_t key[NB];
        uint4 kk[NB];
        uint32_t revbits = 0, actbits = 0;
#pragma unroll
        for (int c = 0; c < NB; ++c) {
            key[c] = 0;
            kk[c] = make_uint4(0, 0, 0, 0);
            if ((uint32_t)c * 64u < K) {
                const bool act = (uint32_t)c * 64u + lane < K;
                bool rev;
                uint32_t qs, qe;
                batch_keys<Spec>(mzh, mzp, (uint32_t)c * 64u, act, key[c], rev, qs, qe);
                revbits |= (rev ? 1u : 0u) << c;
                if (act) {
                    actbits |= 1u << c;
                    kk[c] = ld_u4(&home_bucket(key[c])->key[0]);
                }
                __builtin_amdgcn_sched_barrier(0);
            }
        }
        hashes_done();
        mq_clk(6);
        uint32_t st;
        probe_all<NB>(key, kk, actbits, st);
#ifdef MQ_STAGE_MAP_SPLIT
        mq_clk(13);
        asm volatile("s_waitcnt vmcnt(0)" ::: "memory");
        mq_clk(14);
#endif
#pragma unroll
        for (int c = 0; c < NB; ++c) {
            if ((uint32_t)c * 64u < K) {
                const uint32_t n = K - (uint32_t)c * 64u < 64u ? K - (uint32_t)c * 64u : 64u;
                const bool act = lane < n;
                const uint32_t i0 = (uint32_t)c * 64u + lane;
                uint32_t qs = 0, qe = 0;
                if (act) {
                    qs = mzp[i0];
                    qe = mzq ? mzq[i0 + k - 1] : mzp[i0 + k - 1] + l - 1u;
                }
                Entry e;
                e.start = kk[c].x;
                e.end = kk[c].y;
                e.offset = kk[c].z;
                e.id_rc = kk[c].w;
                const bool hit = ((st >> (2 * c)) & 3u) == 1u && entry_live(e);
                batch_runs(n, key[c], ((revbits >> c) & 1u) != 0, qs, qe, hit, e);
            }
        }
        mq_clk(7);
    }

    __device__ __forceinline__ void finish_runs() {
        if (c_open) {
            if (lane_id() == 0) put_rec(n_matches, M);
            n_matches++;
            c_open = false;
        }
    }

};

}
```

mapquik_amd/csrc/mq_seed.hpp:

```cpp
#pragma once
#include "mq_device.hpp"
#include "mq_hash.hpp"
#include "mq_wave.hpp"

namespace mq {

constexpr uint32_t SD_SR_RAW = 4096;
#ifndef MQ_SD_MAX_SR
#define MQ_SD_MAX_SR 3
#endif
constexpr uint32_t SD_MAX_SR = MQ_SD_MAX_SR;
constexpr uint32_t SD_TILE_RAW = SD_SR_RAW * SD_MAX_SR;
constexpr uint32_t SD_BLOCKS = SD_TILE_RAW / 64;
constexpr uint32_t SD_CODES_MAX = SD_TILE_RAW + MAX_L - 1;
constexpr uint32_t SD_LC_MAX = (SD_CODES_MAX + 63) / 64;
constexpr uint32_t SD_FLAG_WORDS = (SD_LC_MAX + 31) / 32;
constexpr uint32_t SD_CODES_DW = 4 * ((63 * SD_LC_MAX + 16 * ((SD_LC_MAX + 15) / 16) + MAX_L + 32) / 64 + 1);
static_assert((63 * SD_LC_MAX + 16 * ((SD_LC_MAX + 15) / 16) + MAX_L + 32) / 16 < SD_CODES_DW, "code stream read-ahead padding");
static_assert(2 * SD_CODES_MAX / 32 + 2 < SD_CODES_DW, "stage A writes three dwords from a piece pair's first");
#ifndef MQ_SD_OWNER_CAP
#define MQ_SD_OWNER_CAP 256
#endif
#ifndef MQ_SD_CROSS_PREFETCH
#define MQ_SD_CROSS_PREFETCH 1
#endif
constexpr bool SD_CROSS_PREFETCH = MQ_SD_CROSS_PREFETCH != 0;
constexpr uint32_t SD_OWNER_CAP = MQ_SD_OWNER_CAP;
static_assert(SD_BLOCKS <= 256, "block_of holds block numbers in a byte");

struct SeedTables {
    uint4 rot[32 * 16];
    uint4 rem[64];
    uint4 quad[256];
    uint16_t lut[1024];
};

constexpr uint32_t SD_BLOCK_OF_BYTES = (SD_CODES_MAX / 64 + 3 + 15) / 16 * 16;
struct SeedLds {
    uint32_t codes[SD_CODES_DW];
    uint8_t block_of[SD_BLOCK_OF_BYTES];
    unsigned long long heads[SD_BLOCKS];
    uint16_t cnt[SD_BLOCKS + 4];
    uint32_t flagw[SD_FLAG_WORDS * 64];
    uint32_t carry_codes[4];
    uint32_t carry_pos[64];
    uint16_t cand[SD_OWNER_CAP];
};

__device__ __forceinline__ uint64_t seed_of(uint32_t code, bool h32) {
    const uint64_t s = code == 0 ? 0x3c8bfbb395c60474ULL : code == 1 ? 0x3193c18562a02b4cULL : code == 2 ? 0x295549f54be24456ULL : 0x20323ed082572324ULL;
    return h32 ? dup_low(s) : s;
}

__device__ __forceinline__ void build_seed_tables(SeedTables &T, uint32_t l, bool h32) {
    auto seed_of = [h32](uint32_t code) { return mq::seed_of(code, h32); };
    for (uint32_t i = threadIdx.x; i < 1024; i += blockDim.x) {
        uint32_t prev = i & 3u, out = 0, n = 0, hb = 0;
        for (uint32_t m = 0; m < 4; ++m) {
            const uint32_t c = (i >> (2 + 2 * m)) & 3u;
            if (c != prev) {
                out |= c << (2 * n);
                n++;
                hb |= 1u << m;
            }
            prev = c;
        }
        T.lut[i] = (uint16_t)(out | ((2 * n) << 8) | (hb << 12));
    }
    for (uint32_t i = threadIdx.x; i < 32u * 16u; i += blockDim.x) {
        const uint32_t sft = i >> 4, o = i & 3u, in = (i >> 2) & 3u;
        const uint64_t f = rotr64(rotl64(seed_of(o), l) ^ seed_of(in), sft);
        const uint64_t r = rotl64(rotr64(seed_of(o ^ 2u), 1) ^ rotl64(seed_of(in ^ 2u), l - 1u), sft);
        T.rot[i] = h32 ? make_uint4((uint32_t)f, (uint32_t)r, (uint32_t)f, (uint32_t)r) : make_uint4((uint32_t)f, (uint32_t)(f >> 32), (uint32_t)r, (uint32_t)(r >> 32));
    }
    for (uint32_t i = threadIdx.x; i < 64; i += blockDim.x) {
        uint64_t f = 0, r = 0;
        for (uint32_t m = 0; m < (l & 3u); ++m) {
            const uint32_t c = (i >> (2 * m)) & 3u;
            f = rotl64(f, 1) ^ seed_of(c);
            r = rotr64(r, 1) ^ rotl64(seed_of(c ^ 2u), l - 1u);
        }
        T.rem[i] = make_uint4((uint32_t)f, (uint32_t)(f >> 32), (uint32_t)r, (uint32_t)(r >> 32));
    }
    for (uint32_t i = threadIdx.x; i < 256; i += blockDim.x) {
        uint64_t f = 0, r = 0;
        for (uint32_t m = 0; m < 4; ++m) {
            const uint32_t c = (i >> (2 * m)) & 3u;
            f = rotl64(f, 1) ^ seed_of(c);
            r = rotr64(r, 1) ^ rotl64(seed_of(c ^ 2u), l - 1u);
        }
        T.quad[i] = make_uint4((uint32_t)f, (uint32_t)(f >> 32), (uint32_t)r, (uint32_t)(r >> 32));
    }
}


typedef uint4 __attribute__((aligned(1))) uint4_unaligned;

__device__ __forceinline__ uint32_t pack16(uint32_t t0, uint32_t t1, uint32_t t2, uint32_t t3) {
    uint32_t v = (t0 >> 1) | (t1 << 1) | (t2 << 3) | (t3 << 5);
    uint32_t x = ((v >> 6) ^ v) & 0x00CC00CCu;
    v ^= x ^ (x << 6);
    x = ((v >> 12) ^ v) & 0x0000F0F0u;
    v ^= x ^ (x << 12);
    return v;
}

struct Hash2 {
    uint32_t flo, fhi, rlo, rhi;
    __device__ __forceinline__ void roll(const uint4 tv) {
        const uint32_t nfhi = __builtin_amdgcn_alignbit(fhi, flo, 31), nflo = __builtin_amdgcn_alignbit(flo, fhi, 31);
        const uint32_t nrlo = __builtin_amdgcn_alignbit(rhi, rlo, 1), nrhi = __builtin_amdgcn_alignbit(rlo, rhi, 1);
        flo = nflo ^ tv.x;
        fhi = nfhi ^ tv.y;
        rlo = nrlo ^ tv.z;
        rhi = nrhi ^ tv.w;
    }
};

__device__ __forceinline__ uint4 load_piece(const uint8_t *__restrict__ seq, uint32_t len, uint32_t pos) {
    const uint32_t p = pos < len - 16u ? pos : len - 16u;
    return *reinterpret_cast<const uint4_unaligned *>(seq + p);
}
__device__ __forceinline__ uint4 fix_piece(const uint4 v, uint32_t len, uint32_t pos) {
    if (pos + 16u <= len) return v;
    const uint32_t fill = (v.w >> 24) * 0x01010101u;
    const uint32_t nv = pos < len ? len - pos : 0u;
    const uint32_t s = 16u - nv;
    uint32_t w0 = v.x, w1 = v.y, w2 = v.z, w3 = v.w;
    if (s & 4u) { w0 = w1; w1 = w2; w2 = w3; w3 = fill; }
    if (s & 8u) { w0 = w2; w1 = w3; w2 = fill; w3 = fill; }
    if (s & 16u) { w0 = fill; w1 = fill; w2 = fill; w3 = fill; }
    const uint32_t sb = s & 3u;
    return make_uint4(__builtin_amdgcn_alignbyte(w1, w0, sb), __builtin_amdgcn_alignbyte(w2, w1, sb),
                      __builtin_amdgcn_alignbyte(w3, w2, sb), __builtin_amdgcn_alignbyte(fill, w3, sb));
}

struct APre {
    uint4 nx0, nx1, nx2, nx3;
};
struct SeedView {
    uint32_t first_prev;
    uint32_t elig_end;
    uint32_t pos_add;
    uint32_t more_after;
};
__device__ __forceinline__ void stage_a_request(const uint8_t *__restrict__ seq, uint32_t len, uint32_t raw0, APre &pre) {
    const uint32_t pos = raw0 + lane_id() * 64u;
    pre.nx0 = load_piece(seq, len, pos);
    pre.nx1 = load_piece(seq, len, pos + 16u);
    pre.nx2 = load_piece(seq, len, pos + 32u);
    pre.nx3 = load_piece(seq, len, pos + 48u);
}

__device__ __forceinline__ bool seed_stage_a(const uint8_t *__restrict__ seq, uint32_t len, uint32_t raw0, uint32_t carry_n,
                                             uint32_t &carry_prev, bool use_hpc, bool fold, const SeedTables &T, SeedLds &S, uint32_t &n_codes,
                                             uint32_t &n_blocks, uint32_t &raw_end, APre &pre, bool first_is_head = true) {
    const uint32_t lane = lane_id();
    uint32_t n_sr = (len - raw0 + SD_SR_RAW - 1u) / SD_SR_RAW;
    if (n_sr > SD_MAX_SR) n_sr = SD_MAX_SR;
    const uint32_t tile_end = raw0 + n_sr * SD_SR_RAW;
    uint4 &nx0 = pre.nx0, &nx1 = pre.nx1, &nx2 = pre.nx2, &nx3 = pre.nx3;
    if (!SD_CROSS_PREFETCH && raw0 != 0) stage_a_request(seq, len, raw0, pre);
    static_assert(offsetof(SeedLds, block_of) == sizeof(uint32_t) * SD_CODES_DW && SD_CODES_DW % 4 == 0, "block_of is zeroed with the code stream");
    for (uint32_t i = lane * 4u; i < SD_CODES_DW + SD_BLOCK_OF_BYTES / 4u; i += 256u)
        *reinterpret_cast<uint4 *>(reinterpret_cast<uint32_t *>(&S) + i) = make_uint4(0, 0, 0, 0);
    wave_sync();
    if (lane < 4u && carry_n) S.codes[lane] = S.carry_codes[lane];
    uint32_t b2 = 2u * carry_n;
    uint32_t bad = 0;
    constexpr uint32_t S1 = 0x00430041u, S0 = 0x00470054u;
    for (uint32_t sr = 0; sr < n_sr; ++sr) {
        const uint32_t pos = raw0 + sr * SD_SR_RAW + lane * 64u;
        const bool more_sr = sr + 1u < n_sr || (SD_CROSS_PREFETCH && tile_end < len);
        if (raw0 + (sr + 1u) * SD_SR_RAW > len) {
            nx0 = fix_piece(nx0, len, pos);
            nx1 = fix_piece(nx1, len, pos + 16u);
            nx2 = fix_piece(nx2, len, pos + 32u);
            nx3 = fix_piece(nx3, len, pos + 48u);
        }
#ifdef MQ_STAGE_A_SPLIT
        if (sr == 0) mq_clk(raw0 == 0 ? 10 : 13);
        asm volatile("s_waitcnt vmcnt(0) lgkmcnt(0)" ::: "memory");
        mq_clk(sr == 0 ? (raw0 == 0 ? 0 : 14) : 12);
#endif
        uint32_t p[4];
        (void)more_sr;
        auto decode = [&](uint4 &nx, uint32_t j) {
            const uint32_t t0 = nx.x & 0x06060606u, t1 = nx.y & 0x06060606u, t2 = nx.z & 0x06060606u, t3 = nx.w & 0x06060606u;
            bad |= (__builtin_amdgcn_perm(S0, S1, t0) ^ nx.x) | (__builtin_amdgcn_perm(S0, S1, t1) ^ nx.y) |
                   (__builtin_amdgcn_perm(S0, S1, t2) ^ nx.z) | (__builtin_amdgcn_perm(S0, S1, t3) ^ nx.w);
            p[j] = pack16(t0, t1, t2, t3);
            nx = load_piece(seq, len, pos + SD_SR_RAW + 16u * j);
        };
        decode(nx0, 0);
        decode(nx1, 1);
        decode(nx2, 2);
        decode(nx3, 3);
        uint32_t out[4], n2[4], hb[4];
        if (use_hpc) {
            uint32_t pc = (uint32_t)__builtin_amdgcn_update_dpp(0, (int)(p[3] >> 30), 0x138, 0xf, 0xf, false);
            if (lane == 0) pc = (sr == 0 && raw0 == 0 && first_is_head) ? ((p[0] & 3u) ^ 1u) : carry_prev;
#pragma unroll
            for (int j = 0; j < 4; ++j) {
                const uint32_t q = (p[j] << 2) | pc;
                pc = p[j] >> 30;
                const uint32_t e0 = T.lut[q & 0x3FFu], e1 = T.lut[(q >> 8) & 0x3FFu], e2 = T.lut[(q >> 16) & 0x3FFu], e3 = T.lut[p[j] >> 22];
                uint32_t o = e0 & 0xFFu, sh = (e0 >> 8) & 15u;
                o |= (e1 & 0xFFu) << sh;
                sh += (e1 >> 8) & 15u;
                o |= (e2 & 0xFFu) << sh;
                sh += (e2 >> 8) & 15u;
                o |= (e3 & 0xFFu) << sh;
                out[j] = o;
                n2[j] = sh + ((e3 >> 8) & 15u);
                hb[j] = (e0 >> 12) | ((e1 >> 12) << 4) | ((e2 >> 12) << 8) | ((e3 >> 12) << 12);
            }
        } else {
#pragma unroll
            for (int j = 0; j < 4; ++j) {
                const uint32_t pp = pos + 16u * (uint32_t)j;
                const uint32_t nv = pp < len ? (len - pp < 16u ? len - pp : 16u) : 0u;
                const uint32_t m = nv >= 16u ? 0xFFFFFFFFu : ((1u << (2u * nv)) - 1u);
                out[j] = p[j] & m;
                n2[j] = 2u * nv;
                hb[j] = nv >= 16u ? 0xFFFFu : ((1u << nv) - 1u);
            }
        }
        const uint32_t mine = n2[0] + n2[1] + n2[2] + n2[3];
        const uint32_t incl = wave_incl_scan_u32(mine);
        const uint32_t total = rdlane(incl, 63);
        uint32_t bo = b2 + incl - mine;
        S.cnt[sr * 64u + lane] = (uint16_t)(bo >> 1);
        {
            const uint32_t c0 = bo >> 1, c1 = (bo + mine) >> 1, m = (c0 + 63u) & ~63u;
            if (m < c1) S.block_of[m >> 6] = (uint8_t)(sr * 64u + lane);
        }
        S.heads[sr * 64u + lane] = (unsigned long long)(hb[0] | (hb[1] << 16)) | ((unsigned long long)(hb[2] | (hb[3] << 16)) << 32);
        auto put_pair = [&](uint32_t o_a, uint32_t n_a, uint32_t o_b, uint32_t bit) {
            const uint64_t v = (uint64_t)o_a | ((uint64_t)o_b << n_a);
            const uint32_t sh = bit & 31u;
            const uint64_t x = (uint64_t)(uint32_t)v << sh, y = (v >> 32) << sh;
            uint32_t *dst = &S.codes[bit >> 5];
            atomicOr(dst, (uint32_t)x);
            atomicOr(dst + 1, (uint32_t)(x >> 32) | (uint32_t)y);
            atomicOr(dst + 2, (uint32_t)(y >> 32));
        };
        put_pair(out[0], n2[0], out[1], bo);
        put_pair(out[2], n2[2], out[3], bo + n2[0] + n2[1]);
        b2 += total;
        carry_prev = rdlane(p[3], 63) >> 30;
#ifdef MQ_STAGE_A_SPLIT
        mq_clk(15);
#endif
    }
    n_blocks = n_sr * 64u;
    raw_end = raw0 + n_sr * SD_SR_RAW < len ? raw0 + n_sr * SD_SR_RAW : len;
    n_codes = b2 >> 1;
    if (lane == 0) S.cnt[n_blocks] = (uint16_t)n_codes;
    wave_sync();
    return __ballot((bad & (fold ? 0xDFDFDFDFu : 0xFFFFFFFFu)) != 0) == 0;
}

template <uint32_t L>
__device__ __forceinline__ Hash2 window_hash_fixed(const SeedTables &T, const SeedLds &S, uint32_t a) {
    constexpr uint32_t NDW = (L + 15u) / 16u, NQ = L / 4u, REM = L & 3u;
    uint32_t c[NDW + 1];
#pragma unroll
    for (uint32_t m = 0; m <= NDW; ++m) c[m] = S.codes[(a >> 4) + m];
    uint32_t dw[NDW];
#pragma unroll
    for (uint32_t m = 0; m < NDW; ++m) dw[m] = __builtin_amdgcn_alignbit(c[m + 1], c[m], 2u * (a & 15u));
    uint4 tv[NQ + 1];
#pragma unroll
    for (uint32_t q = 0; q < NQ; ++q) tv[q] = T.quad[(dw[q >> 2] >> (8u * (q & 3u))) & 0xFFu];
    if (REM) tv[NQ] = T.rem[(dw[NQ >> 2] >> (8u * (NQ & 3u))) & ((1u << (2u * REM)) - 1u)];
    Hash2 h = {tv[0].x, tv[0].y, tv[0].z, tv[0].w};
#pragma unroll
    for (uint32_t q = 1; q < NQ; ++q) {
        const uint32_t nfhi = __builtin_amdgcn_alignbit(h.fhi, h.flo, 28), nflo = __builtin_amdgcn_alignbit(h.flo, h.fhi, 28);
        const uint32_t nrlo = __builtin_amdgcn_alignbit(h.rhi, h.rlo, 4), nrhi = __builtin_amdgcn_alignbit(h.rlo, h.rhi, 4);
        h.flo = nflo ^ tv[q].x;
        h.fhi = nfhi ^ tv[q].y;
        h.rlo = nrlo ^ tv[q].z;
        h.rhi = nrhi ^ tv[q].w;
    }
    if (REM) {
        const uint32_t nfhi = __builtin_amdgcn_alignbit(h.fhi, h.flo, 32u - REM), nflo = __builtin_amdgcn_alignbit(h.flo, h.fhi, 32u - REM);
        const uint32_t nrlo = __builtin_amdgcn_alignbit(h.rhi, h.rlo, REM), nrhi = __builtin_amdgcn_alignbit(h.rlo, h.rhi, REM);
        h.flo = nflo ^ tv[NQ].x;
        h.fhi = nfhi ^ tv[NQ].y;
        h.rlo = nrlo ^ tv[NQ].z;
        h.rhi = nrhi ^ tv[NQ].w;
    }
    return h;
}

template <uint32_t NQ>
__device__ __forceinline__ Hash2 window_hash_q(const SeedTables &T, const SeedLds &S, uint32_t l, uint32_t a) {
    constexpr uint32_t NDW = (4u * NQ + 3u + 15u) / 16u;
    const uint32_t rem = l & 3u;
    uint32_t c[NDW + 1];
#pragma unroll
    for (uint32_t m = 0; m <= NDW; ++m) c[m] = S.codes[(a >> 4) + m];
    uint32_t dw[NDW];
#pragma unroll
    for (uint32_t m = 0; m < NDW; ++m) dw[m] = __builtin_amdgcn_alignbit(c[m + 1], c[m], 2u * (a & 15u));
    uint4 tv[NQ + 1];
#pragma unroll
    for (uint32_t q = 0; q < NQ; ++q) tv[q] = T.quad[(dw[q >> 2] >> (8u * (q & 3u))) & 0xFFu];
    tv[NQ] = T.rem[(dw[NQ >> 2] >> (8u * (NQ & 3u))) & ((1u << (2u * rem)) - 1u)];
    Hash2 h = {tv[0].x, tv[0].y, tv[0].z, tv[0].w};
#pragma unroll
    for (uint32_t q = 1; q < NQ; ++q) {
        const uint32_t nfhi = __builtin_amdgcn_alignbit(h.fhi, h.flo, 28), nflo = __builtin_amdgcn_alignbit(h.flo, h.fhi, 28);
        const uint32_t nrlo = __builtin_amdgcn_alignbit(h.rhi, h.rlo, 4), nrhi = __builtin_amdgcn_alignbit(h.rlo, h.rhi, 4);
        h.flo = nflo ^ tv[q].x;
        h.fhi = nfhi ^ tv[q].y;
        h.rlo = nrlo ^ tv[q].z;
        h.rhi = nrhi ^ tv[q].w;
    }
    if (rem) {
        const uint32_t nfhi = __builtin_amdgcn_alignbit(h.fhi, h.flo, 32u - rem), nflo = __builtin_amdgcn_alignbit(h.flo, h.fhi, 32u - rem);
        const uint32_t nrlo = __builtin_amdgcn_alignbit(h.rhi, h.rlo, rem), nrhi = __builtin_amdgcn_alignbit(h.rlo, h.rhi, rem);
        h.flo = nflo ^ tv[NQ].x;
        h.fhi = nfhi ^ tv[NQ].y;
        h.rlo = nrlo ^ tv[NQ].z;
        h.rhi = nrhi ^ tv[NQ].w;
    }
    return h;
}

template <class Spec = SpecNone>
__device__ __forceinline__ Hash2 window_hash(const SeedTables &T, const SeedLds &S, uint32_t l, uint32_t a) {
    if constexpr (Spec::FIXED) return window_hash_fixed<Spec::L>(T, S, a);
    if (l == 31u) return window_hash_fixed<31>(T, S, a);
    switch (l >> 2) {
        case 3: return window_hash_q<3>(T, S, l, a);
        case 4: return window_hash_q<4>(T, S, l, a);
        case 5: return window_hash_q<5>(T, S, l, a);
        case 6: return window_hash_q<6>(T, S, l, a);
        case 7: return window_hash_q<7>(T, S, l, a);
// ... 206 lines not shown
                : "+v"(g), "+v"(h), "+v"(fbits) : "v"(e.x), "v"(e.y), "v"(mhi), "s"(bhi) : "vcc");
            const uint32_t s4 = (TT + 5u) & 31u;
            tv[t & 3u] = (t + 4u < 16u) ? rot_at(s4, off16(xe, xo, t + 4u)) : rot_at(s4, off16(xe_n, xo_n, t + 4u - 16u));
        }
    }
    if (LIM_CHECK) fbits <<= 16u - lim;
    return fbits;
}

__device__ __forceinline__ void seed_stage_b32(const SeedTables &T, SeedLds &S, const DevParams &P, uint32_t w_eff) {
    const uint32_t lane = lane_id();
    const uint32_t l = P.l;
    const uint32_t lc = (w_eff + 63u) >> 6;
    const uint32_t s0 = lane * lc;
    const uint32_t bhi = (uint32_t)(P.bound >> 32);
    if (s0 < w_eff) {
        const Hash2 h0 = window_hash(T, S, l, s0);
        uint32_t g = h0.flo, h = h0.rlo;
        auto mk_xe = [](uint32_t ow, uint32_t iw) { return (ow & 0x33333333u) | ((iw & 0x33333333u) << 2); };
        auto mk_xo = [](uint32_t ow, uint32_t iw) { return ((ow >> 2) & 0x33333333u) | (iw & 0xCCCCCCCCu); };
        auto nib = [](uint32_t xe, uint32_t xo, uint32_t s) { return (((s & 1u) ? xo : xe) >> (4u * (s >> 1))) & 0xFu; };
        const uint32_t o_dw = s0 >> 4, o_sh = 2u * (s0 & 15u);
        const uint32_t i_dw = (s0 + l) >> 4, i_sh = 2u * ((s0 + l) & 15u);
        uint32_t prev_o = S.codes[o_dw], prev_i = S.codes[i_dw];
        uint32_t xe, xo;
        {
            const uint32_t no = S.codes[o_dw + 1u], ni = S.codes[i_dw + 1u];
            const uint32_t ow = __builtin_amdgcn_alignbit(no, prev_o, o_sh), iw = __builtin_amdgcn_alignbit(ni, prev_i, i_sh);
            prev_o = no;
            prev_i = ni;
            xe = mk_xe(ow, iw);
            xo = mk_xo(ow, iw);
        }
        uint2 tv[4];
#pragma unroll
        for (uint32_t s = 0; s < 4; ++s) {
            const uint4 e = T.rot[(s + 1u) * 16u + nib(xe, xo, s)];
            tv[s] = make_uint2(e.x, e.y);
        }
        const uint32_t nb = (lc + 15u) >> 4;
        auto next_x = [&](uint32_t b, uint32_t &xe_n, uint32_t &xo_n) {
            const uint32_t no = S.codes[o_dw + b + 2u], ni = S.codes[i_dw + b + 2u];
            const uint32_t ow = __builtin_amdgcn_alignbit(no, prev_o, o_sh), iw = __builtin_amdgcn_alignbit(ni, prev_i, i_sh);
            prev_o = no;
            prev_i = ni;
            xe_n = mk_xe(ow, iw);
            xo_n = mk_xo(ow, iw);
        };
        auto put = [&](uint32_t w_at, uint32_t v) { S.flagw[w_at * 64u + lane] = v; };
        uint32_t blk = 0;
        for (const uint32_t full = (lc >> 5) << 1; blk < full; blk += 2u) {
            uint32_t xe1, xo1, xe2, xo2;
            next_x(blk, xe1, xo1);
            const uint32_t b0 = stage_b_block32<0, false>(T, g, h, tv, xe, xo, xe1, xo1, bhi, 16u);
            next_x(blk + 1u, xe2, xo2);
            const uint32_t b1 = stage_b_block32<1, false>(T, g, h, tv, xe1, xo1, xe2, xo2, bhi, 16u);
            put(blk >> 1, (__brev(b0) >> 16) | (__brev(b1) & 0xFFFF0000u));
            xe = xe2;
            xo = xo2;
        }
        uint32_t word = 0;
        for (; blk < nb; ++blk) {
            uint32_t xe_n, xo_n;
            next_x(blk, xe_n, xo_n);
            const uint32_t lim = lc - 16u * blk;
            uint32_t fbits;
            if (lim >= 16u) {
                fbits = (blk & 1u) ? stage_b_block32<1, false>(T, g, h, tv, xe, xo, xe_n, xo_n, bhi, 16u) : stage_b_block32<0, false>(T, g, h, tv, xe, xo, xe_n, xo_n, bhi, 16u);
            } else {
                fbits = (blk & 1u) ? stage_b_block32<1, true>(T, g, h, tv, xe, xo, xe_n, xo_n, bhi, lim) : stage_b_block32<0, true>(T, g, h, tv, xe, xo, xe_n, xo_n, bhi, lim);
            }
            if (blk & 1u) {
                put(blk >> 1, word | (__brev(fbits) & 0xFFFF0000u));
            } else {
                word = __brev(fbits) >> 16;
            }
            xe = xe_n;
            xo = xo_n;
        }
        if (nb & 1u) put(nb >> 1, word);
    }
}

__device__ __forceinline__ uint32_t select_bit64(unsigned long long m, uint32_t r) {
    uint32_t mw = (uint32_t)m, bit = 0;
    const uint32_t c = (uint32_t)__popc(mw);
    if (r >= c) {
        r -= c;
        mw = (uint32_t)(m >> 32);
        bit = 32;
    }
#pragma unroll
    for (uint32_t width = 16; width >= 1; width >>= 1) {
        const uint32_t half = (uint32_t)__popc(mw & ((1u << width) - 1u));
        if (r >= half) {
            r -= half;
            mw >>= width;
            bit += width;
        }
    }
    return bit;
}

__device__ __forceinline__ uint32_t seed_rawpos_batch(const SeedLds &S, uint32_t raw_base, uint32_t carry_n, uint32_t j) {
    const uint32_t cpos = S.carry_pos[j < 63u ? j : 63u];
    const uint32_t b0 = S.block_of[j >> 6];
    const uint32_t b1 = b0 + 1u < SD_BLOCKS ? b0 + 1u : SD_BLOCKS - 1u, b2 = b0 + 2u < SD_BLOCKS ? b0 + 2u : SD_BLOCKS - 1u;
    const uint32_t c0 = S.cnt[b0], c1 = S.cnt[b0 + 1u], c2 = S.cnt[b0 + 2u], c3 = S.cnt[b0 + 3u];
    const unsigned long long h0 = S.heads[b0], h1 = S.heads[b1], h2 = S.heads[b2];
    const bool s1 = c1 <= j, s2 = s1 && c2 <= j, s3 = s2 && c3 <= j;
    uint32_t b = b0 + (s1 ? 1u : 0u) + (s2 ? 1u : 0u);
    unsigned long long hd = s2 ? h2 : s1 ? h1 : h0;
    uint32_t cb = s2 ? c2 : s1 ? c1 : c0;
    if (__ballot(s3 && j >= carry_n)) {
        if (s3 && j >= carry_n) {
            b = b0 + 3u;
            while ((uint32_t)S.cnt[b + 1u] <= j) ++b;
            hd = S.heads[b];
            cb = S.cnt[b];
        }
    }
    const uint32_t pos = raw_base + b * 64u + select_bit64(hd, j - cb);
    return j < carry_n ? cpos : pos;
}

struct GlobalList {
    unsigned long long *__restrict__ hash;
    uint32_t *__restrict__ pos;
    uint32_t cap;
    uint32_t *__restrict__ last;
    __device__ __forceinline__ void put(uint32_t dest, uint64_t hv, uint32_t p, uint32_t lp) const {
        if (dest < cap) {
            hash[dest] = hv;
            pos[dest] = p;
            if (last) last[dest] = lp;
        }
    }
};
template <bool VIEW = false, class Out = GlobalList, bool VAR = true, class Spec = SpecNone>
__device__ __forceinline__ uint32_t seed_stage_r(const SeedTables &T, SeedLds &S, const DevParams &P, uint32_t w_eff,
                                                 uint32_t n_blocks, uint32_t n_codes, uint32_t raw_base, uint32_t carry_n,
                                                 const Out &out, uint32_t out_base, bool &inexact, const SeedView &V = SeedView()) {
    const uint32_t lane = lane_id();
    const uint32_t lc = (w_eff + 63u) >> 6;
    uint32_t n_listed = 0;
    constexpr uint32_t NW = SD_FLAG_WORDS;
    const uint32_t s0 = lane * lc;
    const uint32_t nv = s0 < w_eff ? (w_eff - s0 < lc ? w_eff - s0 : lc) : 0u;
    uint32_t f[NW];
    uint32_t my_count = 0;
#pragma unroll
    for (uint32_t w = 0; w < NW; ++w) f[w] = S.flagw[w * 64u + lane];
#pragma unroll
    for (uint32_t w = 0; w < NW; ++w) {
        const uint32_t k = nv > 32u * w ? nv - 32u * w : 0u;
        f[w] &= (k >= 32u ? ~0u : ((1u << k) - 1u));
        my_count += (uint32_t)__popc(f[w]);
    }
    const uint32_t incl = wave_incl_scan_u32(my_count);
    const uint32_t total = rdlane(incl, 63);
    const uint32_t my_prefix = incl - my_count;
    const uint32_t nw_used = (lc + 31u) >> 5;
#ifdef MQ_STAGE_R_SPLIT
    mq_clk(12);
#endif
    for (uint32_t r0 = 0; r0 < total; r0 += SD_OWNER_CAP) {
        uint32_t at = my_prefix - r0;
#pragma unroll
        for (uint32_t w = 0; w < NW; ++w) {
            if (w < nw_used) {
                uint32_t g = f[w];
                while (__ballot(g != 0u)) {
                    const bool has = g != 0u;
                    const uint32_t t = s0 + 32u * w + (uint32_t)__ffs((int)g) - 1u;
                    if (has && at < SD_OWNER_CAP) S.cand[at] = (uint16_t)t;
                    at += has ? 1u : 0u;
                    g &= g - 1u;
                }
            }
        }
        wave_sync();
#ifdef MQ_STAGE_R_SPLIT
        mq_clk(13);
#endif
        const uint32_t r1 = total - r0 < SD_OWNER_CAP ? total : r0 + SD_OWNER_CAP;
        for (uint32_t i0 = r0; i0 < r1; i0 += 64u) {
            const uint32_t i = i0 + lane;
            if (i < r1) {
                const uint32_t j = S.cand[i - r0];
                const Hash2 wh = window_hash<Spec>(T, S, spec_l<Spec>(P), j);
#ifdef MQ_STAGE_R_SPLIT
                asm volatile("s_waitcnt lgkmcnt(0)" ::: "memory");
                asm volatile("" ::"v"(wh.flo), "v"(wh.fhi), "v"(wh.rlo), "v"(wh.rhi));
                mq_clk(14);
#endif
                const uint32_t pos = seed_rawpos_batch(S, raw_base, carry_n, j);
                const uint64_t F = ((uint64_t)wh.fhi << 32) | wh.flo, R = ((uint64_t)wh.rhi << 32) | wh.rlo;
                const uint64_t hv = F < R ? F : R;
                if (hv > P.bound) inexact = true;
                const uint32_t dest = out_base + i;
                const bool listed = !VIEW || pos < V.elig_end;
                uint32_t rep = pos, lp = 0;
                if (var_pos_end<VAR>(P)) rep = seed_rawpos_batch(S, raw_base, carry_n, j + 1u) - 1u;
                if (var_end_compressed<VAR>(P)) lp = seed_rawpos_batch(S, raw_base, carry_n, j + spec_l<Spec>(P) - 1u) + (VIEW ? V.pos_add : 0u);
                if (listed) out.put(dest, list_hash<VAR>(P, hv), VIEW ? rep + V.pos_add : rep, lp);
                if (VIEW) n_listed += (uint32_t)__popcll(__ballot(listed));
            }
#ifdef MQ_STAGE_R_SPLIT
            mq_clk(15);
#endif
        }
        wave_sync();
    }
    inexact = __ballot(inexact) != 0;
    return VIEW ? rdfirst(n_listed) : total;
}

constexpr uint32_t SD_NOT_FAST = 0xFFFFFFFFu;
__device__ __forceinline__ bool seed_fast_eligible(uint64_t len) { return len >= 16u && (len >> 32) == 0; }
template <int STOP = 0, bool VIEW = false, class Out = GlobalList, bool VAR = true, class Spec = SpecNone>
__device__ __forceinline__ uint32_t seed_sequence_fast_to(const uint8_t *__restrict__ seq, uint32_t len, const DevParams &P, const SeedTables &T,
                                                          SeedLds &S, const Out &out, APre &pre, bool pre_valid, const SeedView &V = SeedView()) {
    const uint32_t lane = lane_id();
    const uint32_t l = spec_l<Spec>(P);
    uint32_t raw0 = 0, carry_n = 0, carry_prev = VIEW ? (V.first_prev & 3u) : 0u, n_out = 0;
    uint32_t halo_heads = 0, seg_heads = 0;
    if (!seed_fast_eligible(len)) return SD_NOT_FAST;
    if (!pre_valid) stage_a_request(seq, len, 0, pre);
    while (raw0 < len) {
        uint32_t n_codes = 0, n_blocks = 0, raw_end = 0;
        const bool ok = seed_stage_a(seq, len, raw0, carry_n, carry_prev, spec_hpc<Spec>(P), spec_fold<Spec>(P), T, S, n_codes, n_blocks, raw_end, pre,
                                     !VIEW || V.first_prev >= 4u);
        mq_clk(0);
        if (!ok) return SD_NOT_FAST;
        if (VIEW && V.more_after) {
            uint32_t c = 0, c0 = 0;
            for (uint32_t k = lane; k < n_blocks; k += 64u) {
                const uint32_t n = (uint32_t)__popcll(S.heads[k]);
                if (raw0 + 64u * k >= V.elig_end) c += n;
                else c0 += n;
            }
            halo_heads += wave_sum_u32(c);
            seg_heads += wave_sum_u32(c0);
        }
        const bool more = raw_end < len;
        if (STOP != 1 && n_codes >= l) {
            const uint32_t w_eff = n_codes - l + 1u;
            if (var_h32<VAR>(P)) seed_stage_b32(T, S, P, w_eff);
            else seed_stage_b<Spec>(T, S, P, w_eff);
            mq_clk(1);
            if (STOP != 2) {
                bool inexact = false;
                n_out += seed_stage_r<VIEW, Out, VAR, Spec>(T, S, P, w_eff, n_blocks, n_codes, raw0, carry_n, out, n_out, inexact, V);
                mq_clk(2);
                if (inexact) return SD_NOT_FAST;
            }
        }
        if (more) {
            const uint32_t new_cn = n_codes < l - 1u ? n_codes : l - 1u;
            uint32_t cpos = 0, ccode = 0;
            if (lane < new_cn) cpos = seed_rawpos_batch(S, raw0, carry_n, n_codes - new_cn + lane);
            if (lane < 4u) {
                const uint32_t sb = 2u * (n_codes - new_cn) + 32u * lane;
                ccode = __builtin_amdgcn_alignbit(S.codes[(sb >> 5) + 1u], S.codes[sb >> 5], sb & 31u);
                const uint32_t keep = 2u * new_cn > 32u * lane ? 2u * new_cn - 32u * lane : 0u;
                ccode = keep >= 32u ? ccode : (ccode & ((1u << keep) - 1u));
            }
            wave_sync();
            if (lane < new_cn) S.carry_pos[lane] = cpos;
            if (lane < 4u) S.carry_codes[lane] = ccode;
            carry_n = new_cn;
        }
        wave_sync();
        raw0 = raw_end;
        mq_clk(3);
    }
    if (VIEW && V.more_after && halo_heads + 1u < l && seg_heads != 0u) return SD_NOT_FAST;
    return n_out;
}
template <int STOP = 0, bool VIEW = false, bool VAR = true, class Spec = SpecNone>
__device__ __forceinline__ uint32_t seed_sequence_fast(const uint8_t *__restrict__ seq, uint32_t len, const DevParams &P, const SeedTables &T,
                                                       SeedLds &S, unsigned long long *__restrict__ mz_hash,
                                                       uint32_t *__restrict__ mz_pos, uint32_t out_cap, APre &pre, bool pre_valid,
                                                       const SeedView &V = SeedView(), uint32_t *__restrict__ mz_last = nullptr) {
    const GlobalList out = {mz_hash, mz_pos, out_cap, VAR ? mz_last : nullptr};
    return seed_sequence_fast_to<STOP, VIEW, GlobalList, VAR, Spec>(seq, len, P, T, S, out, pre, pre_valid, V);
}

}
```

Baseline: 1368.

## Defer raw position decoding to matched minimizers via per-wave head map

Adds a lazy-position seeding path. Seeding stores compressed code indices instead of raw base positions, and it records per-block head bitmaps and prefix counts in a per-wave global head map. Raw positions are then recovered by select-bit only for the query endpoints of matches. This removes the per-minimizer seed_rawpos_batch work and the carry-position bookkeeping. In exchange it adds global writes of the head map during stage A, extra scratch memory per wave, and more kernel instantiations. It is restricted to the frozen variant-0 pairs with no anchors or chains.

Result: slower. 1304 (-4.7%).

```diff
diff --git a/include/mapquik_hip_diag.h b/include/mapquik_hip_diag.h
--- a/include/mapquik_hip_diag.h
+++ b/include/mapquik_hip_diag.h
@@ -11,6 +11,10 @@
 
 int mqdiag_last_map_spec(mq_index *idx, uint32_t *spec_id);
 int mqdiag_ctx_last_map_spec(mq_ctx *ctx, uint32_t *spec_id);
+
+int mqdiag_last_lazy_pos(mq_index *idx, uint32_t *lazy);
+int mqdiag_ctx_last_lazy_pos(mq_ctx *ctx, uint32_t *lazy);
+uint32_t mqdiag_lazy_max_bases(void);
 
 int mq_last_map_order(mq_index *idx, uint32_t *n_flagged, uint32_t *n_first);
 
diff --git a/mapquik_amd/api.py b/mapquik_amd/api.py
--- a/mapquik_amd/api.py
+++ b/mapquik_amd/api.py
@@ -210,6 +210,11 @@
     if hasattr(L, "mqdiag_last_map_spec"):
         L.mqdiag_last_map_spec.argtypes = [vp, C.POINTER(C.c_uint32)]
         L.mqdiag_ctx_last_map_spec.argtypes = [vp, C.POINTER(C.c_uint32)]
+    if hasattr(L, "mqdiag_last_lazy_pos"):
+        L.mqdiag_last_lazy_pos.argtypes = [vp, C.POINTER(C.c_uint32)]
+        L.mqdiag_ctx_last_lazy_pos.argtypes = [vp, C.POINTER(C.c_uint32)]
+        L.mqdiag_lazy_max_bases.restype = C.c_uint32
+        L.mqdiag_lazy_max_bases.argtypes = []
     if path is None:
         _lib = L
     return L
@@ -559,6 +564,12 @@
         if self._L.mqdiag_last_map_spec(self._h, C.byref(a)) != 0:
             raise _err(self._L, "mqdiag_last_map_spec")
         return a.value
+
+    def last_lazy_pos(self):
+        a = C.c_uint32()
+        if self._L.mqdiag_last_lazy_pos(self._h, C.byref(a)) != 0:
+            raise _err(self._L, "mqdiag_last_lazy_pos")
+        return bool(a.value)
 
     def table_alloc_ms(self):
         ms = C.c_float()
@@ -765,6 +776,12 @@
             raise _err(self._L, "mqdiag_ctx_last_map_spec")
         return a.value
 
+    def last_lazy_pos(self):
+        a = C.c_uint32()
+        if self._L.mqdiag_ctx_last_lazy_pos(self._h, C.byref(a)) != 0:
+            raise _err(self._L, "mqdiag_ctx_last_lazy_pos")
+        return bool(a.value)
+
 
 def format_coverage_bed(index, refs, intervals):
     out = []
diff --git a/mapquik_amd/csrc/mq_capi_diag.hpp b/mapquik_amd/csrc/mq_capi_diag.hpp
--- a/mapquik_amd/csrc/mq_capi_diag.hpp
+++ b/mapquik_amd/csrc/mq_capi_diag.hpp
@@ -112,6 +112,26 @@
     });
 }
 
+int mqdiag_last_lazy_pos(mq_index *idx, uint32_t *lazy) {
+    return guarded([&]() -> int {
+        if (!idx || !lazy) return set_err(MQ_EINVAL, "bad arguments");
+        std::lock_guard<std::mutex> lk(idx->mu);
+        mq_ctx *c = idx->def_ctx.get();
+        if (!c->ev_valid) return set_err(MQ_ESTATE, "no map launch recorded");
+        *lazy = c->last_lazy ? 1u : 0u;
+        return MQ_OK;
+    });
+}
+int mqdiag_ctx_last_lazy_pos(mq_ctx *ctx, uint32_t *lazy) {
+    return guarded([&]() -> int {
+        if (!ctx || !lazy) return set_err(MQ_EINVAL, "bad arguments");
+        if (!ctx->ev_valid) return set_err(MQ_ESTATE, "no map launch recorded");
+        *lazy = ctx->last_lazy ? 1u : 0u;
+        return MQ_OK;
+    });
+}
+uint32_t mqdiag_lazy_max_bases(void) { return LAZY_MAX_BASES; }
+
 int mq_last_map_order(mq_index *idx, uint32_t *n_flagged, uint32_t *n_first) {
     return guarded([&]() -> int {
         if (!idx || !n_flagged || !n_first) return set_err(MQ_EINVAL, "bad arguments");
diff --git a/mapquik_amd/csrc/mq_capi_index.hpp b/mapquik_amd/csrc/mq_capi_index.hpp
--- a/mapquik_amd/csrc/mq_capi_index.hpp
+++ b/mapquik_amd/csrc/mq_capi_index.hpp
@@ -37,6 +37,7 @@
         idx->device = device;
         if (env_int("MQ_CHAIN_CHUNK", 64) == 4) idx->chain_chunk = 4;
         idx->no_spec = env_int("MQ_NO_SPEC", 0) != 0;
+        idx->eager_pos = env_int("MQ_EAGER_POS", 0) != 0;
         set_dev_params(idx.get(), dev_params_from(*params, (params->flags & MQ_FLAG_SEED_VARIANT_MASK) >> MQ_FLAG_SEED_VARIANT_SHIFT));
         idx->force_general = env_int("MQ_FORCE_GENERAL", 0) != 0;
         idx->heavy_first = env_int("MQ_HEAVY_FIRST", 1) != 0;
diff --git a/mapquik_amd/csrc/mq_capi_map.hpp b/mapquik_amd/csrc/mq_capi_map.hpp
--- a/mapquik_amd/csrc/mq_capi_map.hpp
+++ b/mapquik_amd/csrc/mq_capi_map.hpp
@@ -67,6 +67,8 @@
     A.stats64 = &c->d_counter.p->probe;
     A.work = c->work;
     A.heavy_first = idx->heavy_first ? 1u : 0u;
+    const bool lazy = delivers && !anch && !chn && !o.redo && !o.scratch_override && !c->redo && !oc->redo && c->head_map.p != nullptr;
+    A.head_map = lazy ? c->head_map.p : nullptr;
     A.anchors.pool = anch ? oc->anchors.pool.p : nullptr;
     A.anchors.cap = anch ? (uint32_t)oc->anchors.cap : 0u;
     A.anchors.counters = anch ? oc->anchors.counters.p : nullptr;
@@ -90,7 +92,7 @@
         if (o.grid_override) grid = std::min(grid, o.grid_override);
         if (anch || chn) grid = std::min(grid, idx->grid_fused_outputs);
         const dim3 blk(64 * MAP_WAVES);
-        const MapPair &kp = map_pair_of(idx, o.instrumented, &c->last_spec, anch, chn);
+        const MapPair &kp = map_pair_of(idx, o.instrumented, &c->last_spec, anch, chn, lazy, &c->last_lazy);
         hipLaunchKernelGGL(kp.map, dim3(grid), blk, 0, st, A);
         HIPCHK(hipGetLastError());
         hipLaunchKernelGGL(kp.declined, dim3(grid), blk, 0, st, A);
diff --git a/mapquik_amd/csrc/mq_host_state.hpp b/mapquik_amd/csrc/mq_host_state.hpp
--- a/mapquik_amd/csrc/mq_host_state.hpp
+++ b/mapquik_amd/csrc/mq_host_state.hpp
@@ -75,8 +75,10 @@
     ScopedEvent ev0, ev1;
     bool ev_valid = false;
     uint32_t last_spec = 0;
+    bool last_lazy = false;
     Buf<MapCounters> d_counter;
     Buf<MatchRec> scratch;
+    Buf<unsigned long long> head_map;
     size_t scratch_waves = 0;
     Buf<unsigned long long> mz_hash;
     Buf<uint32_t> mz_pos;
@@ -334,6 +336,7 @@
     int chain_chunk = 64;
     bool no_spec = false;
     uint32_t map_spec = 0;
+    bool eager_pos = false;
     double t_add_ms = 0;
     double table_alloc_ms = 0;
     CtxPtr def_ctx;
@@ -506,13 +509,18 @@
                                                         {MQ_OUT_PAIRS(true, false), MQ_OUT_PAIRS(true, true)}};
 #undef MQ_OUT_PAIRS
 
+template <class Spec>
+constexpr MapPair lazy_pair() {
+    return {map_kernel<64, false, false, Spec, false, false, true>, map_declined_kernel<64, false, false, Spec>};
+}
+static const MapPair MAP_LAZY_NONE = lazy_pair<SpecNone>();
 struct MapSpec {
     uint32_t k, l, use_hpc, fold, fast_kh;
-    MapPair pair;
+    MapPair pair, lazy;
 };
 template <class S>
 constexpr MapSpec map_spec() {
-    return {S::K, S::L, S::HPC ? 1u : 0u, S::FOLD ? 1u : 0u, S::FAST_KH ? 1u : 0u, map_pair<64, false, false, S>()};
+    return {S::K, S::L, S::HPC ? 1u : 0u, S::FOLD ? 1u : 0u, S::FAST_KH ? 1u : 0u, map_pair<64, false, false, S>(), lazy_pair<S>()};
 }
 static const MapSpec MAP_SPECS[] = {map_spec<SpecFixed<5, 31, true, false>>(), map_spec<SpecFixed<7, 31, true, false>>(),
                                     map_spec<SpecFixed<5, 31, true, true>>()};
@@ -528,13 +536,20 @@
         if (spec_matches(MAP_SPECS[i], idx->dp, false)) return i + 1;
     return 0;
 }
-static const MapPair &map_pair_of(const mq_index *idx, bool instrumented, uint32_t *spec_id = nullptr, bool anchors = false, bool chains = false) {
+static bool lazy_allowed(const mq_index *idx) { return !idx->eager_pos && idx->dp.variant == 0 && idx->chain_chunk != 4; }
+static const MapPair &map_pair_of(const mq_index *idx, bool instrumented, uint32_t *spec_id = nullptr, bool anchors = false, bool chains = false,
+                                  bool lazy = false, bool *lazy_taken = nullptr) {
+    if (lazy_taken) *lazy_taken = false;
     if ((anchors || chains) && !instrumented) {
         if (spec_id) *spec_id = 0;
         return MAP_KERNELS_OUTPUTS[anchors][chains][idx->dp.variant != 0][idx->chain_chunk == 4];
     }
     const uint32_t sid = instrumented ? 0u : idx->map_spec;
     if (spec_id) *spec_id = sid;
+    if (lazy && !instrumented && lazy_allowed(idx)) {
+        if (lazy_taken) *lazy_taken = true;
+        return sid ? MAP_SPECS[sid - 1].lazy : MAP_LAZY_NONE;
+    }
     return sid ? MAP_SPECS[sid - 1].pair : MAP_KERNELS[idx->dp.variant != 0][instrumented][idx->chain_chunk == 4];
 }
 static void set_dev_params(mq_index *idx, const DevParams &dp) {
@@ -556,6 +571,12 @@
     if (specs_allowed(idx))
         for (const MapSpec &s : MAP_SPECS)
             if (spec_matches(s, idx->dp, true)) pairs.push_back(s.pair);
+    if (lazy_allowed(idx)) {
+        pairs.push_back(MAP_LAZY_NONE);
+        if (specs_allowed(idx))
+            for (const MapSpec &s : MAP_SPECS)
+                if (spec_matches(s, idx->dp, true)) pairs.push_back(s.lazy);
+    }
     for (const MapPair &kp : pairs)
         for (const MapFn fn : {kp.map, kp.declined}) {
             if ((rc = occ_of((const void *)fn, 64 * MAP_WAVES, occ))) return rc;
@@ -629,6 +650,7 @@
             c->scratch_waves = 0;
             const size_t nw = std::min(max_waves, want + want / 4);
             if ((rc = c->scratch.alloc(nw * idx->cap_matches))) return rc;
+            if (lazy_allowed(idx) && (rc = c->head_map.alloc(nw * LAZY_WAVE_WORDS))) return rc;
             c->scratch_waves = nw;
         }
     }
diff --git a/mapquik_amd/csrc/mq_lazy_pos.hpp b/mapquik_amd/csrc/mq_lazy_pos.hpp
--- /dev/null
+++ b/mapquik_amd/csrc/mq_lazy_pos.hpp
@@ -0,0 +1,80 @@
+#pragma once
+#include <stdint.h>
+
+#if defined(__HIPCC__) || defined(__CUDACC__)
+#define MQ_HD __host__ __device__ __forceinline__
+#else
+#define MQ_HD inline
+#endif
+
+namespace mq {
+
+#ifndef MQ_LAZY_MAX_BASES
+#define MQ_LAZY_MAX_BASES 524288
+#endif
+constexpr uint32_t LAZY_MAX_BASES = MQ_LAZY_MAX_BASES;
+static_assert(LAZY_MAX_BASES >= 4096 && LAZY_MAX_BASES % 4096 == 0, "whole super-rows");
+constexpr uint32_t LAZY_BLOCKS = LAZY_MAX_BASES / 64;
+constexpr uint32_t LAZY_ROWS = LAZY_BLOCKS + 4;
+constexpr uint32_t LAZY_WAVE_WORDS = 2 * LAZY_ROWS;
+struct LazyMap {
+    unsigned long long *base = nullptr;
+    MQ_HD unsigned long long *heads() const { return base; }
+    MQ_HD uint32_t *first() const { return reinterpret_cast<uint32_t *>(base + LAZY_ROWS); }
+    MQ_HD uint32_t *block_of() const { return first() + LAZY_ROWS; }
+};
+
+MQ_HD uint32_t lazy_ld(const uint32_t *p) {
+#if defined(__HIP_DEVICE_COMPILE__)
+    return __hip_atomic_load(p, __ATOMIC_RELAXED, __HIP_MEMORY_SCOPE_AGENT);
+#else
+    return *p;
+#endif
+}
+MQ_HD unsigned long long lazy_ld(const unsigned long long *p) {
+#if defined(__HIP_DEVICE_COMPILE__)
+    return __hip_atomic_load(p, __ATOMIC_RELAXED, __HIP_MEMORY_SCOPE_AGENT);
+#else
+    return *p;
+#endif
+}
+
+MQ_HD uint32_t select_bit64(unsigned long long m, uint32_t r) {
+    uint32_t mw = (uint32_t)m, bit = 0;
+    const uint32_t c = (uint32_t)__builtin_popcount(mw);
+    if (r >= c) {
+        r -= c;
+        mw = (uint32_t)(m >> 32);
+        bit = 32;
+    }
+#pragma unroll
+    for (uint32_t width = 16; width >= 1; width >>= 1) {
+        const uint32_t half = (uint32_t)__builtin_popcount(mw & ((1u << width) - 1u));
+        if (r >= half) {
+            r -= half;
+            mw >>= width;
+            bit += width;
+        }
+    }
+    return bit;
+}
+
+MQ_HD uint32_t lazy_rawpos(const unsigned long long *heads, const uint32_t *first, const uint32_t *block_of, uint32_t g) {
+    const uint32_t b0 = lazy_ld(block_of + (g >> 6));
+    const uint32_t c0 = lazy_ld(first + b0), c1 = lazy_ld(first + b0 + 1u), c2 = lazy_ld(first + b0 + 2u), c3 = lazy_ld(first + b0 + 3u);
+    const unsigned long long h0 = lazy_ld(heads + b0), h1 = lazy_ld(heads + b0 + 1u), h2 = lazy_ld(heads + b0 + 2u);
+    const bool s1 = c1 <= g, s2 = s1 && c2 <= g, s3 = s2 && c3 <= g;
+    uint32_t b = b0 + (s1 ? 1u : 0u) + (s2 ? 1u : 0u);
+    unsigned long long hd = s2 ? h2 : s1 ? h1 : h0;
+    uint32_t cb = s2 ? c2 : s1 ? c1 : c0;
+    if (s3) {
+        b = b0 + 3u;
+        while (lazy_ld(first + b + 1u) <= g) ++b;
+        hd = lazy_ld(heads + b);
+        cb = lazy_ld(first + b);
+    }
+    return b * 64u + select_bit64(hd, g - cb);
+}
+MQ_HD uint32_t lazy_rawpos(const LazyMap &hm, uint32_t g) { return lazy_rawpos(hm.heads(), hm.first(), hm.block_of(), g); }
+
+}
diff --git a/mapquik_amd/csrc/mq_map_kernels.hpp b/mapquik_amd/csrc/mq_map_kernels.hpp
--- a/mapquik_amd/csrc/mq_map_kernels.hpp
+++ b/mapquik_amd/csrc/mq_map_kernels.hpp
@@ -32,6 +32,7 @@
     AnchorOut anchors;
     mq_anchor_span *anchor_spans;
     const uint32_t *anchor_ids;
+    unsigned long long *head_map;
 };
 
 __device__ __forceinline__ uint32_t *read_cycles(const MapArgs &A) { return A.mz_count; }
@@ -97,14 +98,16 @@
     return at + cnt <= A.pool_cap;
 }
 
-template <int STOP = 0, bool VAR = true, class Spec = SpecNone>
+template <int STOP = 0, bool VAR = true, class Spec = SpecNone, bool LAZY = false>
 __device__ __forceinline__ uint32_t seed_read_fast(const MapArgs &A, const SeedTables &T, SeedLds &S, const uint8_t *seq,
-                                                   uint32_t len, uint64_t &base, uint32_t cap, uint32_t &n_moved, APre &pre, bool pre_valid) {
-    uint32_t cnt = seed_sequence_fast<STOP, false, VAR, Spec>(seq, len, A.P, T, S, A.mz_hash + base, A.mz_pos + base, cap, pre, pre_valid, SeedView(),
-                                                        A.mz_last ? A.mz_last + base : nullptr);
+                                                   uint32_t len, uint64_t &base, uint32_t cap, uint32_t &n_moved, APre &pre, bool pre_valid,
+                                                   const LazyMap &hm = LazyMap()) {
+    uint32_t cnt = seed_sequence_fast<STOP, false, VAR, Spec, LAZY>(seq, len, A.P, T, S, A.mz_hash + base, A.mz_pos + base, cap, pre, pre_valid, SeedView(),
+                                                              A.mz_last ? A.mz_last + base : nullptr, hm);
     if (cnt != SD_NOT_FAST && cnt > cap) {
         if (pool_take(A, cnt, base)) {
-            seed_sequence_fast<0, false, VAR, Spec>(seq, len, A.P, T, S, A.mz_hash + base, A.mz_pos + base, cnt, pre, false, SeedView(), A.mz_last ? A.mz_last + base : nullptr);
+            seed_sequence_fast<0, false, VAR, Spec, LAZY>(seq, len, A.P, T, S, A.mz_hash + base, A.mz_pos + base, cnt, pre, false, SeedView(),
+                                                          A.mz_last ? A.mz_last + base : nullptr, hm);
             n_moved++;
         } else {
             cnt = LIST_OVERFLOW;
@@ -354,10 +357,12 @@
     return A.counters->chains.windows + (size_t)wave_gid * A.counters->chains.win_cap;
 }
 
-template <int CH, bool TIMING, bool VAR = true, class Spec = SpecNone, bool ANCH = false, bool CHN = false>
+template <int CH, bool TIMING, bool VAR = true, class Spec = SpecNone, bool ANCH = false, bool CHN = false, bool LAZY = false>
 __device__ __forceinline__ void map_read(const MapArgs &A, MapListLds &S, MatchRec *scratch, uint32_t r, uint64_t len, uint32_t cnt,
                                          uint64_t base, unsigned long long &t_steps, unsigned long long &t_lookups, mq_hit &h,
-                                         mq_anchor_span *sp = nullptr, ChainRec *cwin = nullptr, mq_chain_span *csp = nullptr) {
+                                         mq_anchor_span *sp = nullptr, ChainRec *cwin = nullptr, mq_chain_span *csp = nullptr,
+                                         const LazyMap &hm = LazyMap()) {
+    static_assert(!LAZY || (!VAR && !ANCH && !CHN), "compressed indices: the product pairs only");
     const uint32_t lane = lane_id();
     const DevParams &P = A.P;
     const uint32_t k = spec_k<Spec>(P);
@@ -406,7 +411,7 @@
             wave_sync();
             mq_clk(5);
             uint32_t *mzq = (VAR && A.mz_last) ? reinterpret_cast<uint32_t *>(S.h) : nullptr;
-            sink.template consume_list<ML_NB, Spec>(S.h, S.p, have, [&]() {
+            sink.template consume_list<ML_NB, Spec, LAZY>(S.h, S.p, have, [&]() {
                 if (mzq) {
                     const uint32_t *lq = A.mz_last + base + g;
                     wave_sync();
@@ -423,6 +428,12 @@
             wave_sync();
             MatchRec m0 = {};
             if (lane_id() < sink.n_matches) m0 = S.rec[lane_id()];
+            if constexpr (LAZY) {
+                if (lane_id() < sink.n_matches) {
+                    m0.q_start = lazy_rawpos(hm, m0.q_start);
+                    m0.q_end = lazy_rawpos(hm, m0.q_end) + spec_l<Spec>(P) - 1u;
+                }
+            }
             mq_clk(8);
             if constexpr (CHN) chain_stage<CH, ANCH, true>(S.rec, sink.n_matches, P, len, A.ref_lens, h, &m0, &A.anchors, sp, &A.counters->chains, cwin, csp);
             else if constexpr (ANCH) chain_stage<CH, true>(S.rec, sink.n_matches, P, len, A.ref_lens, h, &m0, &A.anchors, sp);
@@ -437,6 +448,15 @@
             } else if (sink.n_matches > 0) {
                 asm volatile("s_waitcnt vmcnt(0)" ::: "memory");
                 wave_sync();
+                if constexpr (LAZY) {
+                    for (uint32_t i = lane; i < sink.n_matches; i += 64u) {
+                        const uint32_t qs = lazy_rawpos(hm, scratch[i].q_start), qe = lazy_rawpos(hm, scratch[i].q_end) + spec_l<Spec>(P) - 1u;
+                        scratch[i].q_start = qs;
+                        scratch[i].q_end = qe;
+                    }
+                    asm volatile("s_waitcnt vmcnt(0)" ::: "memory");
+                    wave_sync();
+                }
                 mq_clk(8);
                 if constexpr (CHN) chain_stage<CH, ANCH, true>(scratch, sink.n_matches, P, len, A.ref_lens, h, nullptr, &A.anchors, sp, &A.counters->chains, cwin, csp);
                 else if constexpr (ANCH) chain_stage<CH, true>(scratch, sink.n_matches, P, len, A.ref_lens, h, nullptr, &A.anchors, sp);
@@ -466,8 +486,9 @@
     MapListLds map;
 };
 
-template <int CH, bool TIMING = false, bool VAR = false, class Spec = SpecNone, bool ANCH = false, bool CHN = false>
+template <int CH, bool TIMING = false, bool VAR = false, class Spec = SpecNone, bool ANCH = false, bool CHN = false, bool LAZY = false>
 __global__ __launch_bounds__(64 * MAP_WAVES, MQ_MAP_MIN_WAVES) void map_kernel(const MapArgs A) {
+    static_assert(!LAZY || (CH == 64 && !TIMING && !VAR && !ANCH && !CHN), "LAZY: the product pairs only");
     __shared__ struct {
         SeedTables T;
         MapWaveLds SS[MAP_WAVES];
@@ -481,6 +502,8 @@
     MapWaveLds &S = SS[wv];
     const size_t wave_gid = (size_t)blockIdx.x * MAP_WAVES + wv;
     MatchRec *scratch = A.scratch_all + wave_gid * A.cap_matches;
+    LazyMap hm;
+    if constexpr (LAZY) hm.base = A.head_map + wave_gid * LAZY_WAVE_WORDS;
     const DevParams &P = A.P;
     const uint64_t o_base = A.offsets[0];
     uint32_t n_fast = 0, n_general = 0, n_moved = 0;
@@ -540,6 +563,8 @@
         } else if (len >= (uint64_t)spec_l<Spec>(P) + spec_k<Spec>(P) - 1u && !var_keep_none<VAR>(P)) {
             uint32_t cap;
             list_region(A, o0 - o_base, len, r, base, cap);
+            if constexpr (LAZY) cnt = (A.force_general || len > LAZY_MAX_BASES) ? SD_NOT_FAST : seed_read_fast<0, VAR, Spec, true>(A, T, S.seed, A.bases + o0, (uint32_t)len, base, cap, n_moved, pre, false, hm);
+            else
             cnt = A.force_general ? SD_NOT_FAST : seed_read_fast<0, VAR, Spec>(A, T, S.seed, A.bases + o0, (uint32_t)len, base, cap, n_moved, pre, false);
             if (cnt == SD_NOT_FAST) {
                 n_general++;
@@ -561,6 +586,7 @@
         mq_chain_span csp;
         if constexpr (CHN) map_read<CH, TIMING, VAR, Spec, ANCH, true>(A, S.map, scratch, r, len, cnt, base, t_steps, t_lookups, h, &sp, chain_window(A, wave_gid), &csp);
         else if constexpr (ANCH) map_read<CH, TIMING, VAR, Spec, true>(A, S.map, scratch, r, len, cnt, base, t_steps, t_lookups, h, &sp);
+        else if constexpr (LAZY) map_read<CH, TIMING, VAR, Spec, false, false, true>(A, S.map, scratch, r, len, cnt, base, t_steps, t_lookups, h, nullptr, nullptr, nullptr, hm);
         else map_read<CH, TIMING, VAR, Spec>(A, S.map, scratch, r, len, cnt, base, t_steps, t_lookups, h);
         wave_sync();
         const uint32_t r_done = r;
diff --git a/mapquik_amd/csrc/mq_probe.hpp b/mapquik_amd/csrc/mq_probe.hpp
--- a/mapquik_amd/csrc/mq_probe.hpp
+++ b/mapquik_amd/csrc/mq_probe.hpp
@@ -264,7 +264,7 @@
         }
     }
 
-    template <int NB, class Spec = SpecNone, class F>
+    template <int NB, class Spec = SpecNone, bool LAZY = false, class F>
     __device__ __forceinline__ void consume_list(const unsigned long long *mzh, const uint32_t *mzp, uint32_t have, const F &hashes_done,
                                                  const uint32_t *mzq = nullptr) {
         const uint32_t k = spec_k<Spec>(P), l = spec_l<Spec>(P);
@@ -309,7 +309,8 @@
                 uint32_t qs = 0, qe = 0;
                 if (act) {
                     qs = mzp[i0];
-                    qe = mzq ? mzq[i0 + k - 1] : mzp[i0 + k - 1] + l - 1u;
+                    if constexpr (LAZY) qe = mzp[i0 + k - 1];
+                    else qe = mzq ? mzq[i0 + k - 1] : mzp[i0 + k - 1] + l - 1u;
                 }
                 Entry e;
                 e.start = kk[c].x;
diff --git a/mapquik_amd/csrc/mq_seed.hpp b/mapquik_amd/csrc/mq_seed.hpp
--- a/mapquik_amd/csrc/mq_seed.hpp
+++ b/mapquik_amd/csrc/mq_seed.hpp
@@ -1,6 +1,7 @@
 #pragma once
 #include "mq_device.hpp"
 #include "mq_hash.hpp"
+#include "mq_lazy_pos.hpp"
 #include "mq_wave.hpp"
 
 namespace mq {
@@ -152,9 +153,11 @@
     pre.nx3 = load_piece(seq, len, pos + 48u);
 }
 
+template <bool LAZY = false>
 __device__ __forceinline__ bool seed_stage_a(const uint8_t *__restrict__ seq, uint32_t len, uint32_t raw0, uint32_t carry_n,
                                              uint32_t &carry_prev, bool use_hpc, bool fold, const SeedTables &T, SeedLds &S, uint32_t &n_codes,
-                                             uint32_t &n_blocks, uint32_t &raw_end, APre &pre, bool first_is_head = true) {
+                                             uint32_t &n_blocks, uint32_t &raw_end, APre &pre, bool first_is_head = true,
+                                             const LazyMap &hm = LazyMap(), uint32_t cbase = 0) {
     const uint32_t lane = lane_id();
     uint32_t n_sr = (len - raw0 + SD_SR_RAW - 1u) / SD_SR_RAW;
     if (n_sr > SD_MAX_SR) n_sr = SD_MAX_SR;
@@ -236,6 +239,13 @@
             if (m < c1) S.block_of[m >> 6] = (uint8_t)(sr * 64u + lane);
         }
         S.heads[sr * 64u + lane] = (unsigned long long)(hb[0] | (hb[1] << 16)) | ((unsigned long long)(hb[2] | (hb[3] << 16)) << 32);
+        if constexpr (LAZY) {
+            const uint32_t gb = (raw0 >> 6) + sr * 64u + lane;
+            const uint32_t g0 = cbase + (bo >> 1), g1 = cbase + ((bo + mine) >> 1), m = (g0 + 63u) & ~63u;
+            hm.heads()[gb] = (unsigned long long)(hb[0] | (hb[1] << 16)) | ((unsigned long long)(hb[2] | (hb[3] << 16)) << 32);
+            hm.first()[gb] = g0;
+            if (m < g1) hm.block_of()[m >> 6] = gb;
+        }
         auto put_pair = [&](uint32_t o_a, uint32_t n_a, uint32_t o_b, uint32_t bit) {
             const uint64_t v = (uint64_t)o_a | ((uint64_t)o_b << n_a);
             const uint32_t sh = bit & 31u;
@@ -257,6 +267,9 @@
     raw_end = raw0 + n_sr * SD_SR_RAW < len ? raw0 + n_sr * SD_SR_RAW : len;
     n_codes = b2 >> 1;
     if (lane == 0) S.cnt[n_blocks] = (uint16_t)n_codes;
+    if constexpr (LAZY) {
+        if (lane == 0) hm.first()[(raw0 >> 6) + n_blocks] = cbase + n_codes;
+    }
     wave_sync();
     return __ballot((bad & (fold ? 0xDFDFDFDFu : 0xFFFFFFFFu)) != 0) == 0;
 }
@@ -629,25 +642,6 @@
     }
 }
 
-__device__ __forceinline__ uint32_t select_bit64(unsigned long long m, uint32_t r) {
-    uint32_t mw = (uint32_t)m, bit = 0;
-    const uint32_t c = (uint32_t)__popc(mw);
-    if (r >= c) {
-        r -= c;
-        mw = (uint32_t)(m >> 32);
-        bit = 32;
-    }
-#pragma unroll
-    for (uint32_t width = 16; width >= 1; width >>= 1) {
-        const uint32_t half = (uint32_t)__popc(mw & ((1u << width) - 1u));
-        if (r >= half) {
-            r -= half;
-            mw >>= width;
-            bit += width;
-        }
-    }
-    return bit;
-}
 
 __device__ __forceinline__ uint32_t seed_rawpos_batch(const SeedLds &S, uint32_t raw_base, uint32_t carry_n, uint32_t j) {
     const uint32_t cpos = S.carry_pos[j < 63u ? j : 63u];
@@ -684,10 +678,11 @@
         }
     }
 };
-template <bool VIEW = false, class Out = GlobalList, bool VAR = true, class Spec = SpecNone>
+template <bool VIEW = false, class Out = GlobalList, bool VAR = true, class Spec = SpecNone, bool LAZY = false>
 __device__ __forceinline__ uint32_t seed_stage_r(const SeedTables &T, SeedLds &S, const DevParams &P, uint32_t w_eff,
                                                  uint32_t n_blocks, uint32_t n_codes, uint32_t raw_base, uint32_t carry_n,
-                                                 const Out &out, uint32_t out_base, bool &inexact, const SeedView &V = SeedView()) {
+                                                 const Out &out, uint32_t out_base, bool &inexact, const SeedView &V = SeedView(), uint32_t cbase = 0) {
+    static_assert(!LAZY || (!VIEW && !VAR), "compressed indices: whole reads of the frozen reading only");
     const uint32_t lane = lane_id();
     const uint32_t lc = (w_eff + 63u) >> 6;
     uint32_t n_listed = 0;
@@ -741,7 +736,9 @@
                 asm volatile("" ::"v"(wh.flo), "v"(wh.fhi), "v"(wh.rlo), "v"(wh.rhi));
                 mq_clk(14);
 #endif
-                const uint32_t pos = seed_rawpos_batch(S, raw_base, carry_n, j);
+                uint32_t pos;
+                if constexpr (LAZY) pos = cbase + j;
+                else pos = seed_rawpos_batch(S, raw_base, carry_n, j);
                 const uint64_t F = ((uint64_t)wh.fhi << 32) | wh.flo, R = ((uint64_t)wh.rhi << 32) | wh.rlo;
                 const uint64_t hv = F < R ? F : R;
                 if (hv > P.bound) inexact = true;
@@ -765,19 +762,21 @@
 
 constexpr uint32_t SD_NOT_FAST = 0xFFFFFFFFu;
 __device__ __forceinline__ bool seed_fast_eligible(uint64_t len) { return len >= 16u && (len >> 32) == 0; }
-template <int STOP = 0, bool VIEW = false, class Out = GlobalList, bool VAR = true, class Spec = SpecNone>
+template <int STOP = 0, bool VIEW = false, class Out = GlobalList, bool VAR = true, class Spec = SpecNone, bool LAZY = false>
 __device__ __forceinline__ uint32_t seed_sequence_fast_to(const uint8_t *__restrict__ seq, uint32_t len, const DevParams &P, const SeedTables &T,
-                                                          SeedLds &S, const Out &out, APre &pre, bool pre_valid, const SeedView &V = SeedView()) {
+                                                          SeedLds &S, const Out &out, APre &pre, bool pre_valid, const SeedView &V = SeedView(),
+                                                          const LazyMap &hm = LazyMap()) {
     const uint32_t lane = lane_id();
     const uint32_t l = spec_l<Spec>(P);
     uint32_t raw0 = 0, carry_n = 0, carry_prev = VIEW ? (V.first_prev & 3u) : 0u, n_out = 0;
     uint32_t halo_heads = 0, seg_heads = 0;
+    uint32_t cbase = 0;
     if (!seed_fast_eligible(len)) return SD_NOT_FAST;
     if (!pre_valid) stage_a_request(seq, len, 0, pre);
     while (raw0 < len) {
         uint32_t n_codes = 0, n_blocks = 0, raw_end = 0;
-        const bool ok = seed_stage_a(seq, len, raw0, carry_n, carry_prev, spec_hpc<Spec>(P), spec_fold<Spec>(P), T, S, n_codes, n_blocks, raw_end, pre,
-                                     !VIEW || V.first_prev >= 4u);
+        const bool ok = seed_stage_a<LAZY>(seq, len, raw0, carry_n, carry_prev, spec_hpc<Spec>(P), spec_fold<Spec>(P), T, S, n_codes, n_blocks, raw_end, pre,
+                                           !VIEW || V.first_prev >= 4u, hm, cbase);
         mq_clk(0);
         if (!ok) return SD_NOT_FAST;
         if (VIEW && V.more_after) {
@@ -798,7 +797,7 @@
             mq_clk(1);
             if (STOP != 2) {
                 bool inexact = false;
-                n_out += seed_stage_r<VIEW, Out, VAR, Spec>(T, S, P, w_eff, n_blocks, n_codes, raw0, carry_n, out, n_out, inexact, V);
+                n_out += seed_stage_r<VIEW, Out, VAR, Spec, LAZY>(T, S, P, w_eff, n_blocks, n_codes, raw0, carry_n, out, n_out, inexact, V, cbase);
                 mq_clk(2);
                 if (inexact) return SD_NOT_FAST;
             }
@@ -806,7 +805,9 @@
         if (more) {
             const uint32_t new_cn = n_codes < l - 1u ? n_codes : l - 1u;
             uint32_t cpos = 0, ccode = 0;
-            if (lane < new_cn) cpos = seed_rawpos_batch(S, raw0, carry_n, n_codes - new_cn + lane);
+            if constexpr (!LAZY) {
+                if (lane < new_cn) cpos = seed_rawpos_batch(S, raw0, carry_n, n_codes - new_cn + lane);
+            }
             if (lane < 4u) {
                 const uint32_t sb = 2u * (n_codes - new_cn) + 32u * lane;
                 ccode = __builtin_amdgcn_alignbit(S.codes[(sb >> 5) + 1u], S.codes[sb >> 5], sb & 31u);
@@ -814,8 +815,11 @@
                 ccode = keep >= 32u ? ccode : (ccode & ((1u << keep) - 1u));
             }
             wave_sync();
-            if (lane < new_cn) S.carry_pos[lane] = cpos;
+            if constexpr (!LAZY) {
+                if (lane < new_cn) S.carry_pos[lane] = cpos;
+            }
             if (lane < 4u) S.carry_codes[lane] = ccode;
+            if constexpr (LAZY) cbase += n_codes - new_cn;
             carry_n = new_cn;
         }
         wave_sync();
@@ -825,13 +829,14 @@
     if (VIEW && V.more_after && halo_heads + 1u < l && seg_heads != 0u) return SD_NOT_FAST;
     return n_out;
 }
-template <int STOP = 0, bool VIEW = false, bool VAR = true, class Spec = SpecNone>
+template <int STOP = 0, bool VIEW = false, bool VAR = true, class Spec = SpecNone, bool LAZY = false>
 __device__ __forceinline__ uint32_t seed_sequence_fast(const uint8_t *__restrict__ seq, uint32_t len, const DevParams &P, const SeedTables &T,
                                                        SeedLds &S, unsigned long long *__restrict__ mz_hash,
                                                        uint32_t *__restrict__ mz_pos, uint32_t out_cap, APre &pre, bool pre_valid,
-                                                       const SeedView &V = SeedView(), uint32_t *__restrict__ mz_last = nullptr) {
+                                                       const SeedView &V = SeedView(), uint32_t *__restrict__ mz_last = nullptr,
+                                                       const LazyMap &hm = LazyMap()) {
     const GlobalList out = {mz_hash, mz_pos, out_cap, VAR ? mz_last : nullptr};
-    return seed_sequence_fast_to<STOP, VIEW, GlobalList, VAR, Spec>(seq, len, P, T, S, out, pre, pre_valid, V);
-}
-
-}
+    return seed_sequence_fast_to<STOP, VIEW, GlobalList, VAR, Spec, LAZY>(seq, len, P, T, S, out, pre, pre_valid, V, hm);
+}
+
+}
```
